# treangenlab/Seqwin

Measured on AMD Instinct MI355X. Metric: Gbp/s minimizer-indexed, higher is better.
Workload: dtype u64

## Files before the change

seqwin_amd/csrc/index.hip:

```cpp
#include <cstdlib>
#include <cstring>
#include <map>
#include <memory>

#include <rocprim/rocprim.hpp>

#include "device.hpp"

namespace sw {

namespace {

constexpr int TPB = 256;
inline unsigned blocks_for(uint64_t n, int per = TPB) { return (unsigned)((n + per - 1) / per); }
inline bool ranks_by_table()
{
    const char *e = SW_TEST_GETENV("SEQWIN_AMD_RANKS");
    return e && !strcmp(e, "table");
}

template <class K, class V>
void sort_pairs(K *&keys, K *&keys_alt, V *&vals, V *&vals_alt, size_t n, unsigned begin_bit, unsigned end_bit,
                hipStream_t stream)
{
    rocprim::double_buffer<K> dk(keys, keys_alt);
    rocprim::double_buffer<V> dv(vals, vals_alt);
    size_t tmp_bytes = 0;
    SW_HIP(rocprim::radix_sort_pairs(nullptr, tmp_bytes, dk, dv, n, begin_bit, end_bit, stream));
    DevArray<unsigned char> tmp(tmp_bytes);
    SW_HIP(rocprim::radix_sort_pairs(tmp.p, tmp_bytes, dk, dv, n, begin_bit, end_bit, stream));
    keys = dk.current();
    keys_alt = dk.alternate();
    vals = dv.current();
    vals_alt = dv.alternate();
}

}

bool sort_keys64_is_own(size_t n)
{
    const char *e = SW_TEST_GETENV("SEQWIN_AMD_SORT");
    const bool own = e ? !strcmp(e, "own") : n >= (1ull << 23);
    return own && !(e && !strcmp(e, "rocprim"));
}

void sort_keys64(uint64_t *&keys, uint64_t *&keys_alt, size_t n, unsigned begin_bit, unsigned end_bit, hipStream_t stream,
                 uint32_t *d_fail, bool perm_hi32, unsigned long long *d_hist_given, unsigned layout_bits)
{
    if (sort_keys64_is_own(n)) {
        radix_sort_keys64(keys, keys_alt, n, begin_bit, end_bit, stream, d_fail, perm_hi32, d_hist_given, layout_bits);
        return;
    }
    rocprim::double_buffer<uint64_t> dk(keys, keys_alt);
    size_t tmp_bytes = 0;
    SW_HIP(rocprim::radix_sort_keys(nullptr, tmp_bytes, dk, n, begin_bit, end_bit, stream));
    DevArray<unsigned char> tmp(tmp_bytes);
    SW_HIP(rocprim::radix_sort_keys(tmp.p, tmp_bytes, dk, n, begin_bit, end_bit, stream));
    keys = dk.current();
    keys_alt = dk.alternate();
}

bool sort_pairs_is_own(size_t n, unsigned bits)
{
    const char *e = SW_TEST_GETENV("SEQWIN_AMD_PAIR_SORT"), *all = SW_TEST_GETENV("SEQWIN_AMD_SORT");
    if (e && !strcmp(e, "rocprim")) return false;
    if (bits % 8 != 0 || bits > 32 || n >= 0xFFFFFFFFull) return false;
    bool own = n >= (1ull << 20);
    if (all) own = !strcmp(all, "own");
    if (e && !strcmp(e, "own")) own = true;
    return own && radix_pairs_available();
}

bool sort_pairs32(uint32_t *&keys, uint32_t *&keys_alt, OccPay *&vals, OccPay *&vals_alt, uint64_t n, unsigned end_bit,
                  hipStream_t stream, uint32_t *d_fail, uint32_t *low_out)
{
    if (sort_pairs_is_own(n, end_bit)) {
        radix_sort_pairs32(keys, keys_alt, vals, vals_alt, n, end_bit, stream, d_fail, nullptr, std::function<void()>(), low_out);
        return low_out != nullptr && n != 0 && end_bit != 0;
    }
    sort_pairs(keys, keys_alt, vals, vals_alt, n, 0, end_bit, stream);
    return false;
}

void check_sort_failed(uint32_t fail_word)
{
    if (fail_word)
        raise(SW_ERR_RUNTIME, "internal error: a radix pass gave up waiting for a lower-numbered workgroup (set SEQWIN_AMD_SORT=rocprim)");
}

namespace {

template <class InIt, class OutIt, class T>
void inclusive_sum(InIt in, OutIt out, size_t n, T, hipStream_t stream)
{
    size_t tmp_bytes = 0;
    SW_HIP(rocprim::inclusive_scan(nullptr, tmp_bytes, in, out, n, rocprim::plus<T>(), stream));
    DevArray<unsigned char> tmp(tmp_bytes);
    SW_HIP(rocprim::inclusive_scan(tmp.p, tmp_bytes, in, out, n, rocprim::plus<T>(), stream));
}

template <class InIt, class OutIt, class T>
void inclusive_sum_keep(InIt in, OutIt out, size_t n, T, hipStream_t stream, DevArray<unsigned char> &tmp)
{
    size_t tmp_bytes = 0;
    SW_HIP(rocprim::inclusive_scan(nullptr, tmp_bytes, in, out, n, rocprim::plus<T>(), stream));
    tmp.alloc(tmp_bytes);
    SW_HIP(rocprim::inclusive_scan(tmp.p, tmp_bytes, in, out, n, rocprim::plus<T>(), stream));
}

template <class InIt, class OutIt, class T>
void exclusive_sum(InIt in, OutIt out, size_t n, T init, hipStream_t stream)
{
    size_t tmp_bytes = 0;
    SW_HIP(rocprim::exclusive_scan(nullptr, tmp_bytes, in, out, init, n, rocprim::plus<T>(), stream));
    DevArray<unsigned char> tmp(tmp_bytes);
    SW_HIP(rocprim::exclusive_scan(tmp.p, tmp_bytes, in, out, init, n, rocprim::plus<T>(), stream));
}

struct U32ToU64 {
    __host__ __device__ uint64_t operator()(uint32_t v) const { return v; }
};

struct HeadFlag {
    const uint64_t *keys;
    uint64_t sentinel;
    __host__ __device__ uint32_t operator()(uint64_t s) const
    {
        const uint64_t k = keys[s];
        return (k != sentinel && (s == 0 || k != keys[s - 1])) ? 1u : 0u;
    }
};

template <bool INDEX, bool RAW = false>
__global__ void k_order(const uint64_t *__restrict__ stage_hash, const uint64_t *__restrict__ stage_kmer,
                        const uint32_t *__restrict__ tile_count, const uint64_t *__restrict__ tile_offset,
                        const uint64_t *__restrict__ dst_off, uint32_t n_tiles, uint64_t mult, uint64_t *__restrict__ hash,
                        uint64_t *__restrict__ kmer, uint32_t *__restrict__ key32, OccPay *__restrict__ pay,
                        uint32_t *__restrict__ rec)
{
    const uint32_t wave = (blockIdx.x * blockDim.x + threadIdx.x) >> 6;
    const uint32_t lane = threadIdx.x & 63u;
    if (wave >= n_tiles) return;
    const uint32_t c = tile_count[wave];
    const uint64_t src = tile_offset[wave], dst = dst_off[wave];
    for (uint32_t i = lane; i < c; i += 64) {
        uint64_t h = stage_hash[src + i];
        if (!RAW) {
            h *= mult;
            h ^= h >> 27;
        }
        const uint64_t km = stage_kmer[src + i];
        if (INDEX) {
            key32[dst + i] = (uint32_t)(h >> 32);
            OccPay p;
            p.low = (uint32_t)h;
            p.pos = (uint32_t)km;
            p.rec = (uint32_t)(km >> 32);
            p.idx = (uint32_t)(dst + i);
            pay[dst + i] = p;
            rec[dst + i] = p.rec;
            if (hash) hash[dst + i] = h;
        } else {
            hash[dst + i] = h;
            kmer[dst + i] = km;
        }
    }
}

__global__ void k_rows_to_pay(const uint64_t *__restrict__ rows, uint64_t n, uint32_t *__restrict__ key32, OccPay *__restrict__ pay)
{
    const uint64_t i = (uint64_t)blockIdx.x * blockDim.x + threadIdx.x;
    if (i >= n) return;
    const uint64_t h = rows[2 * i], km = rows[2 * i + 1];
    key32[i] = (uint32_t)(h >> 32);
    OccPay p;
    p.low = (uint32_t)h;
    p.pos = (uint32_t)km;
    p.rec = (uint32_t)(km >> 32);
    p.idx = (uint32_t)i;
    pay[i] = p;
}

__global__ void k_iota(uint32_t *v, uint64_t n)
{
    const uint64_t i = (uint64_t)blockIdx.x * blockDim.x + threadIdx.x;
    if (i < n) v[i] = (uint32_t)i;
}

#ifndef SW_NODES_ROWS
#define SW_NODES_ROWS 4
#endif
constexpr int NODES_ROWS = SW_NODES_ROWS;
constexpr int NODES_THREADS = 1024;
constexpr int NODES_WAVES = NODES_THREADS / 64;
constexpr uint32_t NODES_ROW = NODES_THREADS * 2;
constexpr uint32_t NODES_TILE = NODES_ROW * NODES_ROWS;
constexpr uint32_t UNSORT_BITS = 14;
constexpr uint32_t UNSORT_RANGE = 1u << UNSORT_BITS;
constexpr bool UNSORT_FUSED_DEFAULT = true;
constexpr uint64_t UNSORT_DIRECT_MAX = 1ull << 25;

constexpr unsigned long long TS_AGG = 1ull << 62, TS_INC = 2ull << 62;

__device__ __forceinline__ unsigned long long interleave32(uint32_t a, uint32_t b)
{
    unsigned long long x = a, y = b;
    x = (x | (x << 16)) & 0x0000FFFF0000FFFFull; y = (y | (y << 16)) & 0x0000FFFF0000FFFFull;
    x = (x | (x << 8)) & 0x00FF00FF00FF00FFull;  y = (y | (y << 8)) & 0x00FF00FF00FF00FFull;
    x = (x | (x << 4)) & 0x0F0F0F0F0F0F0F0Full;  y = (y | (y << 4)) & 0x0F0F0F0F0F0F0F0Full;
    x = (x | (x << 2)) & 0x3333333333333333ull;  y = (y | (y << 2)) & 0x3333333333333333ull;
    x = (x | (x << 1)) & 0x5555555555555555ull;  y = (y | (y << 1)) & 0x5555555555555555ull;
    return x | (y << 1);
}

constexpr uint32_t RANK_REP = 0x80000000u;
constexpr uint8_t OWNER_DROP = 0xFF;
constexpr uint32_t NODES_DIGITS = 256;
struct NodesScat {
    uint64_t stage[NODES_TILE];
    unsigned long long goff[NODES_DIGITS];
    uint32_t cnt[NODES_DIGITS];
    uint32_t lstart[NODES_DIGITS];
};
template <bool BITS, bool REP, bool SCAT = false>
__global__ __launch_bounds__(NODES_THREADS) void k_nodes(const uint32_t *__restrict__ key32, const OccPay *__restrict__ pay, uint64_t n,
                                               uint64_t base, const uint32_t *__restrict__ rec_flag, sw_kmer *__restrict__ kmers,
                                               uint64_t *__restrict__ node_hash, uint32_t *__restrict__ node_start,
                                               uint32_t *__restrict__ rank_direct,
                                               uint64_t *__restrict__ uval,
                                               unsigned long long *__restrict__ tbits, unsigned long long *__restrict__ nbits,
                                               unsigned long long *__restrict__ tile_state, uint32_t *__restrict__ ticket,
                                               uint32_t *__restrict__ n_nodes_out, uint32_t *__restrict__ order_bad,
                                               unsigned long long *__restrict__ cursor, uint32_t dig_shift, uint32_t dig_mask)
{
    __shared__ uint32_t s_tile, s_excl;
    __shared__ uint32_t s_row[NODES_ROWS * NODES_WAVES];
    static_assert(NODES_ROWS * NODES_WAVES <= 128, "the (row, wave) group counts are scanned by one wave, two per lane");
    const uint32_t lane = threadIdx.x & 63u, wave = threadIdx.x >> 6;
    NodesScat *sc = nullptr;
    if constexpr (SCAT) {
        __shared__ NodesScat s_scat;
        sc = &s_scat;
        if (threadIdx.x < NODES_DIGITS) sc->cnt[threadIdx.x] = 0;
    }
    if (threadIdx.x == 0) s_tile = atomicAdd(ticket, 1u);
    __syncthreads();
    const uint32_t tile = s_tile;
    const uint64_t s0 = (uint64_t)tile * NODES_TILE;
    uint32_t k[NODES_ROWS][2], within[NODES_ROWS], headm = 0, prec[NODES_ROWS];
    OccPay p[NODES_ROWS][2];
    unsigned long long misorder = 0;
#pragma unroll
    for (int r = 0; r < NODES_ROWS; ++r) {
        const uint64_t s = s0 + (uint64_t)r * NODES_ROW + 2 * threadIdx.x;
        k[r][0] = k[r][1] = 0;
        p[r][0] = p[r][1] = OccPay{0, 0, 0, 0};
        if (s + 1 < n) {
            const uint2 kk = *reinterpret_cast<const uint2 *>(key32 + s);
            k[r][0] = kk.x;
            k[r][1] = kk.y;
            p[r][0] = pay[s];
            p[r][1] = pay[s + 1];
        } else if (s < n) {
            k[r][0] = key32[s];
            p[r][0] = pay[s];
        }
        uint32_t pk = __shfl_up(k[r][1], 1, 64), plow = __shfl_up(p[r][1].low, 1, 64), pidx = __shfl_up(p[r][1].idx, 1, 64);
        prec[r] = __shfl_up(p[r][1].rec, 1, 64);
        if (lane == 0 && s < n && s) {
            pk = key32[s - 1];
            const OccPay q = pay[s - 1];
            plow = q.low;
            prec[r] = q.rec;
            pidx = q.idx;
        }
        const bool h0 = s < n && (s == 0 || k[r][0] != pk || p[r][0].low != plow);
        const bool h1 = s + 1 < n && (k[r][1] != k[r][0] || p[r][1].low != p[r][0].low);
#ifndef SW_NO_ORDER_GUARD
        {
            const unsigned long long hp = ((unsigned long long)pk << 32) | plow, h0v = ((unsigned long long)k[r][0] << 32) | p[r][0].low,
                                     h1v = ((unsigned long long)k[r][1] << 32) | p[r][1].low;
            const bool bad0 = s < n && s && (h0v < hp || (!h0 && p[r][0].idx <= pidx));
            const bool bad1 = s + 1 < n && (h1v < h0v || (!h1 && p[r][1].idx <= p[r][0].idx));
            misorder |= __ballot(bad0 || bad1);
        }
#else
        (void)pidx;
#endif
        const unsigned long long b0 = __ballot(h0), b1 = __ballot(h1), lt = (1ull << lane) - 1ull;
        within[r] = (uint32_t)__popcll(b0 & lt) + (uint32_t)__popcll(b1 & lt);
        if (h0) headm |= 1u << (2 * r);
        if (h1) headm |= 2u << (2 * r);
        if (lane == 0) s_row[r * NODES_WAVES + wave] = (uint32_t)__popcll(b0) + (uint32_t)__popcll(b1);
    }
    if (misorder && lane == 0) atomicAdd(order_bad, (uint32_t)__popcll(misorder));
    uint32_t drank[NODES_ROWS][2];
    if constexpr (SCAT) {
#pragma unroll
        for (int r = 0; r < NODES_ROWS; ++r)
#pragma unroll
            for (int e = 0; e < 2; ++e) {
                drank[r][e] = 0;
                if (s0 + (uint64_t)r * NODES_ROW + 2 * threadIdx.x + e < n)
                    drank[r][e] = atomicAdd(&sc->cnt[(p[r][e].idx >> dig_shift) & dig_mask], 1u);
            }
    }
    __syncthreads();
    if (SCAT && wave == 1) {
        const uint4 c4 = reinterpret_cast<const uint4 *>(sc->cnt)[lane];
        const uint32_t c[4] = {c4.x, c4.y, c4.z, c4.w};
        unsigned long long g[4];
#pragma unroll
        for (int j = 0; j < 4; ++j)
            g[j] = c[j] ? atomicAdd(&cursor[(size_t)(4 * lane + j) * UNSORT_CURSOR_STRIDE], (unsigned long long)c[j]) : 0ull;
        uint32_t incl = c[0] + c[1] + c[2] + c[3];
        for (uint32_t d = 1; d < 64; d <<= 1) {
            const uint32_t up = __shfl_up(incl, d, 64);
            if (lane >= d) incl += up;
        }
        uint32_t before = incl - (c[0] + c[1] + c[2] + c[3]);
#pragma unroll
        for (int j = 0; j < 4; ++j) {
            sc->lstart[4 * lane + j] = before;
            sc->goff[4 * lane + j] = g[j] - before;
            before += c[j];
        }
    }
    if (wave == 0) {
        constexpr uint32_t GROUPS = NODES_ROWS * NODES_WAVES;
        const uint32_t c0 = (2 * lane < GROUPS) ? s_row[2 * lane] : 0u, c1 = (2 * lane + 1 < GROUPS) ? s_row[2 * lane + 1] : 0u;
        uint32_t incl = c0 + c1;
        for (uint32_t d = 1; d < 64; d <<= 1) {
            const uint32_t up = __shfl_up(incl, d, 64);
            if (lane >= d) incl += up;
        }
        const uint32_t total = __shfl(incl, 63, 64);
        if (2 * lane < GROUPS) s_row[2 * lane] = incl - c0 - c1;
        if (2 * lane + 1 < GROUPS) s_row[2 * lane + 1] = incl - c1;
        if (lane == 0)
            __hip_atomic_store(&tile_state[tile], (tile == 0 ? TS_INC : TS_AGG) | total, __ATOMIC_RELAXED, __HIP_MEMORY_SCOPE_AGENT);
        uint32_t excl = 0;
        if (tile) {
            int64_t look = (int64_t)tile - 1;
            for (;;) {
                const int64_t idx = look - lane;
                const unsigned long long st = idx >= 0 ? __hip_atomic_load(&tile_state[idx], __ATOMIC_RELAXED, __HIP_MEMORY_SCOPE_AGENT)
                                                       : TS_INC;
                const unsigned long long inc = __ballot((st >> 62) == 2), none = __ballot((st >> 62) == 0);
                const uint32_t first_inc = inc ? (uint32_t)__builtin_ctzll(inc) : 64u;
                const unsigned long long needed = first_inc >= 63 ? ~0ull : ((2ull << first_inc) - 1ull);
                if (none & needed) {
                    __builtin_amdgcn_s_sleep(2);
                    continue;
                }
                uint32_t v = (lane <= first_inc) ? (uint32_t)st : 0u;
                for (int d = 32; d; d >>= 1) v += __shfl_xor(v, d, 64);
                excl += v;
                if (first_inc < 64) break;
                look -= 64;
            }
            if (lane == 0)
                __hip_atomic_store(&tile_state[tile], TS_INC | (unsigned long long)(excl + total), __ATOMIC_RELAXED,
                                   __HIP_MEMORY_SCOPE_AGENT);
        }
        if (lane == 0) {
            s_excl = excl;
            if (s0 + NODES_TILE >= n) *n_nodes_out = excl + total;
        }
    }
    __syncthreads();
    const uint32_t excl = s_excl;
    if constexpr (SCAT) {
#pragma unroll
        for (int r = 0; r < NODES_ROWS; ++r)
#pragma unroll
            for (int e = 0; e < 2; ++e) drank[r][e] += sc->lstart[(p[r][e].idx >> dig_shift) & dig_mask];
    }
#pragma unroll
    for (int r = 0; r < NODES_ROWS; ++r) {
        const uint64_t s = s0 + (uint64_t)r * NODES_ROW + 2 * threadIdx.x;
        const bool live0 = s < n, live1 = s + 1 < n;
        const bool h0 = (headm >> (2 * r)) & 1u, h1 = (headm >> (2 * r + 1)) & 1u;
        const uint32_t nid0 = excl + s_row[r * NODES_WAVES + wave] + within[r] + (h0 ? 1u : 0u) - 1u;
        const uint32_t nid1 = nid0 + (h1 ? 1u : 0u);
        uint32_t w0 = nid0, w1 = nid1;
        uint32_t f0 = 0, f1 = 0, pf = 0;
        if (BITS || REP) {
            f0 = live0 ? rec_flag[p[r][0].rec] : 0u;
            f1 = live1 ? rec_flag[p[r][1].rec] : 0u;
            pf = __shfl_up(f1, 1, 64);
            if (lane == 0 && live0 && s) pf = rec_flag[prec[r]];
        }
        if (REP) {
            uint32_t nk = __shfl_down(k[r][0], 1, 64), nlow = __shfl_down(p[r][0].low, 1, 64), nf = __shfl_down(f0, 1, 64);
            bool nlive = __shfl_down((int)live0, 1, 64) != 0;
            if (lane == 63) {
                nlive = s + 2 < n;
                if (nlive) {
                    nk = key32[s + 2];
                    const OccPay q = pay[s + 2];
                    nlow = q.low;
                    nf = rec_flag[q.rec];
                }
            }
            const bool same01 = live1 && !h1 && (f1 >> 1) == (f0 >> 1);
            const bool same_p0 = live0 && !h0 && (f0 >> 1) == (pf >> 1);
            const bool same_1n = live1 && nlive && nk == k[r][1] && nlow == p[r][1].low && (nf >> 1) == (f1 >> 1);
            if (same_p0 || same01) w0 |= RANK_REP;
            if (same01 || same_1n) w1 |= RANK_REP;
        }
        if (live1) {
            *reinterpret_cast<uint4 *>(kmers + s) = make_uint4(p[r][0].pos, p[r][0].rec, p[r][1].pos, p[r][1].rec);
            if (!SCAT && uval)
                *reinterpret_cast<ulonglong2 *>(uval + s) = make_ulonglong2(((uint64_t)p[r][0].idx << 32) | w0,
                                                                          ((uint64_t)p[r][1].idx << 32) | w1);
        } else if (live0) {
            sw_kmer km;
            km.pos = p[r][0].pos;
            km.record_idx = p[r][0].rec;
            kmers[s] = km;
            if (!SCAT && uval) uval[s] = ((uint64_t)p[r][0].idx << 32) | w0;
        }
        if constexpr (SCAT) {
            if (live0) sc->stage[drank[r][0]] = ((uint64_t)p[r][0].idx << 32) | w0;
            if (live1) sc->stage[drank[r][1]] = ((uint64_t)p[r][1].idx << 32) | w1;
        }
        if (rank_direct) {
            if (live0) rank_direct[p[r][0].idx] = w0;
            if (live1) rank_direct[p[r][1].idx] = w1;
        }
#pragma unroll
        for (int e = 0; e < 2; ++e) {
            const bool head = e ? h1 : h0;
            if (head) {
                const uint32_t nid = e ? nid1 : nid0;
                node_hash[nid] = ((uint64_t)k[r][e] << 32) | p[r][e].low;
                node_start[nid] = (uint32_t)(s + e);
            }
        }
        if (BITS) {
            const bool first0 = live0 && (h0 || (f0 >> 1) != (pf >> 1)), first1 = live1 && (h1 || (f1 >> 1) != (f0 >> 1));
            const unsigned long long t0 = __ballot(first0 && (f0 & 1u)), t1 = __ballot(first1 && (f1 & 1u));
            const unsigned long long g0 = __ballot(first0 && !(f0 & 1u)), g1 = __ballot(first1 && !(f1 & 1u));
            if (lane == 0 && live0) {
                const uint64_t wd = s >> 6;
                tbits[wd] = interleave32((uint32_t)t0, (uint32_t)t1);
                nbits[wd] = interleave32((uint32_t)g0, (uint32_t)g1);
                if (s + 64 < n) {
                    tbits[wd + 1] = interleave32((uint32_t)(t0 >> 32), (uint32_t)(t1 >> 32));
                    nbits[wd + 1] = interleave32((uint32_t)(g0 >> 32), (uint32_t)(g1 >> 32));
                }
            }
        }
    }
    if constexpr (SCAT) {
        asm volatile("s_waitcnt lgkmcnt(0)" ::: "memory");
        __builtin_amdgcn_s_barrier();
        asm volatile("" ::: "memory");
        const uint32_t cnt_tile = (uint32_t)min((uint64_t)NODES_TILE, n - s0);
        constexpr int OUT = NODES_TILE / NODES_THREADS;
        uint64_t word[OUT], at[OUT];
#pragma unroll
        for (int j = 0; j < OUT; ++j) word[j] = sc->stage[j * NODES_THREADS + threadIdx.x];
#pragma unroll
        for (int j = 0; j < OUT; ++j) at[j] = sc->goff[(uint32_t)(word[j] >> (32 + dig_shift)) & dig_mask] + (j * NODES_THREADS + threadIdx.x);
#pragma unroll
        for (int j = 0; j < OUT; ++j)
            if (j * NODES_THREADS + threadIdx.x < cnt_tile && at[j] < n) uval[at[j]] = word[j];
    }
}

__device__ __forceinline__ uint32_t popc_range(const unsigned long long *__restrict__ w, uint64_t a, uint64_t b)
{
    if (a >= b) return 0;
    const uint64_t wa = a >> 6, wb = (b - 1) >> 6;
    const unsigned long long ma = ~0ull << (a & 63u), mb = ~0ull >> (63u - ((b - 1) & 63u));
    if (wa == wb) return (uint32_t)__popcll(w[wa] & ma & mb);
    uint32_t c = (uint32_t)__popcll(w[wa] & ma) + (uint32_t)__popcll(w[wb] & mb);
    for (uint64_t i = wa + 1; i < wb; ++i) c += (uint32_t)__popcll(w[i]);
    return c;
}

constexpr int FIN_THREADS = 256;
template <bool BITS>
__global__ __launch_bounds__(FIN_THREADS) void k_finish_nodes(sw_node *__restrict__ nodes, uint64_t n_nodes, const uint64_t *__restrict__ node_hash,
                                                              const uint32_t *__restrict__ node_start, uint64_t base, uint64_t end,
                                                              const unsigned long long *__restrict__ tbits,
                                                              const unsigned long long *__restrict__ nbits, double inv_tar, double inv_neg)
{
    static_assert(sizeof(sw_node) == 40, "five 8-byte words per node");
    __shared__ __align__(16) unsigned long long stage[FIN_THREADS * 5];
    const uint64_t i0 = (uint64_t)blockIdx.x * FIN_THREADS, i = i0 + threadIdx.x;
    if (i < n_nodes) {
        const uint32_t a = node_start[i];
        const uint64_t b = i + 1 < n_nodes ? (uint64_t)node_start[i + 1] : end - base;
        uint32_t n_tar = 0, n_neg = 0;
        double pen = 0.0;
        if (BITS) {
            n_tar = popc_range(tbits, a, b);
            n_neg = popc_range(nbits, a, b);
            {
#pragma clang fp contract(off)
                const double ft = (double)n_tar * inv_tar;
                const double fn = (double)n_neg * inv_neg;
                const double omf = 1.0 - ft;
                const double aa = omf * omf;
                const double bb = fn * fn;
                const double sum = aa + bb;
                pen = __dsqrt_rn(sum);
            }
        }
        unsigned long long *w = stage + threadIdx.x * 5;
        w[0] = node_hash[i];
        w[1] = base + a;
        w[2] = base + b;
        w[3] = ((unsigned long long)n_neg << 32) | n_tar;
        w[4] = (unsigned long long)__double_as_longlong(pen);
    }
    __syncthreads();
    const uint64_t cnt = min((uint64_t)FIN_THREADS, n_nodes - i0);
    const uint32_t n16 = (uint32_t)(cnt * 40 / 16), tail8 = (uint32_t)((cnt * 40) % 16) / 8;
    uint4 *dst = reinterpret_cast<uint4 *>(nodes + i0);
    const uint4 *src = reinterpret_cast<const uint4 *>(stage);
    for (uint32_t t = threadIdx.x; t < n16; t += FIN_THREADS) dst[t] = src[t];
    if (tail8 && threadIdx.x == 0) reinterpret_cast<unsigned long long *>(nodes + i0)[n16 * 2] = stage[n16 * 2];
}

__global__ void k_rec_flag(const uint32_t *__restrict__ rec_asm, const uint8_t *__restrict__ is_target, uint64_t n_records,
                           uint32_t *__restrict__ rec_flag)
{
    const uint64_t r = (uint64_t)blockIdx.x * blockDim.x + threadIdx.x;
    if (r < n_records) {
        const uint32_t a = rec_asm[r];
        rec_flag[r] = (a << 1) | ((is_target && is_target[a]) ? 1u : 0u);
    }
}

constexpr unsigned long long TABLE_EMPTY = ~0ull;
__device__ __forceinline__ uint64_t table_mix(uint64_t x)
{
    return x ^ (x >> 29);
}

__global__ void k_table_build(const sw_node *__restrict__ nodes, uint64_t n_nodes, ulonglong2 *__restrict__ slots, uint64_t mask,
                              uint32_t *__restrict__ rank_of_empty_key)
{
    const uint64_t r = (uint64_t)blockIdx.x * blockDim.x + threadIdx.x;
    if (r >= n_nodes) return;
    const unsigned long long h = nodes[r].hash;
    if (h == TABLE_EMPTY) {
        *rank_of_empty_key = (uint32_t)r;
        return;
    }
    uint64_t s = table_mix(h) & mask;
    for (;;) {
        const unsigned long long old = atomicCAS(&slots[s].x, TABLE_EMPTY, h);
        if (old == TABLE_EMPTY) {
            slots[s].y = r;
            return;
        }
        s = (s + 1) & mask;
    }
}

__global__ void k_table_lookup(const uint64_t *__restrict__ hash, uint64_t n, const ulonglong2 *__restrict__ slots, uint64_t mask,
                               const uint32_t *__restrict__ rank_of_empty_key, uint32_t *__restrict__ rank)
{
    const uint64_t i = (uint64_t)blockIdx.x * blockDim.x + threadIdx.x;
    if (i >= n) return;
    const unsigned long long h = hash[i];
    if (h == TABLE_EMPTY) {
        rank[i] = *rank_of_empty_key;
        return;
    }
    uint64_t s = table_mix(h) & mask;
    for (;;) {
        const ulonglong2 e = slots[s];
        if (e.x == h) {
            rank[i] = (uint32_t)e.y;
            return;
        }
        if (e.x == TABLE_EMPTY) {
            rank[i] = 0xFFFFFFFFu;
            return;
        }
        s = (s + 1) & mask;
    }
}

__global__ __launch_bounds__(1024) void k_unsort_bucket(const uint64_t *__restrict__ uval, uint64_t n, uint32_t *__restrict__ rank)
{
    __shared__ uint32_t sr[UNSORT_RANGE];
    const uint64_t b0 = (uint64_t)blockIdx.x * UNSORT_RANGE;
    const uint32_t cnt = (uint32_t)min((uint64_t)UNSORT_RANGE, n - b0);
#pragma unroll
    for (uint32_t h = 0; h < UNSORT_RANGE / 1024u; h += 8) {
        uint64_t v[8];
#pragma unroll
        for (uint32_t j = 0; j < 8; ++j) {
            const uint32_t t = threadIdx.x + (h + j) * 1024u;
            v[j] = t < cnt ? uval[b0 + t] : 0ull;
        }
#pragma unroll
        for (uint32_t j = 0; j < 8; ++j)
            if (threadIdx.x + (h + j) * 1024u < cnt) sr[(uint32_t)(v[j] >> 32) & (UNSORT_RANGE - 1u)] = (uint32_t)v[j];
    }
    __syncthreads();
    for (uint32_t t = threadIdx.x; t < cnt; t += 1024) rank[b0 + t] = sr[t];
}

__global__ void k_node_starts(const sw_node *__restrict__ nodes, uint64_t n_nodes, uint32_t *__restrict__ start)
{
    const uint64_t i = (uint64_t)blockIdx.x * blockDim.x + threadIdx.x;
    if (i < n_nodes) start[i] = (uint32_t)nodes[i].start;
}

__global__ void k_occ_rows(const sw_kmer *__restrict__ kmers, const sw_node *__restrict__ nodes,
                           const uint32_t *__restrict__ start, uint64_t n_nodes, uint64_t n_kmers, uint64_t rec_offset,
                           uint64_t *__restrict__ rows)
{
    const uint64_t s = (uint64_t)blockIdx.x * blockDim.x + threadIdx.x;
    if (s >= n_kmers) return;
    uint64_t lo = 0, hi = n_nodes;
    while (hi - lo > 1) {
        const uint64_t mid = (lo + hi) >> 1;
        if (start[mid] <= s) lo = mid; else hi = mid;
    }
    rows[2 * s] = nodes[lo].hash;
    rows[2 * s + 1] = (uint64_t)kmers[s].pos | (((uint64_t)kmers[s].record_idx + rec_offset) << 32);
}

__global__ void k_strided_copy(const uint64_t *__restrict__ src, uint32_t stride, uint32_t col, uint64_t n,
                               uint64_t *__restrict__ dst)
{
    const uint64_t i = (uint64_t)blockIdx.x * blockDim.x + threadIdx.x;
    if (i < n) dst[i] = src[i * stride + col];
}

__global__ void k_gather_col(const uint64_t *__restrict__ rows, uint32_t stride, uint32_t col,
                             const uint32_t *__restrict__ idx, uint64_t n, uint64_t *__restrict__ dst)
{
    const uint64_t i = (uint64_t)blockIdx.x * blockDim.x + threadIdx.x;
    if (i < n) dst[i] = rows[(uint64_t)idx[i] * stride + col];
}

__global__ void k_rebase_nodes(sw_node *__restrict__ nodes, uint64_t n_nodes, uint64_t base)
{
    const uint64_t i = (uint64_t)blockIdx.x * blockDim.x + threadIdx.x;
    if (i < n_nodes) {
        nodes[i].start += base;
        nodes[i].stop += base;
    }
}

struct PairHeadFlag {
    const uint64_t *a, *b;
    __host__ __device__ uint32_t operator()(uint64_t s) const
    {
        return (s == 0 || a[s] != a[s - 1] || b[s] != b[s - 1]) ? 1u : 0u;
    }
};

__global__ void k_merge_edge_heads(const uint64_t *__restrict__ f, const uint64_t *__restrict__ sd,
                                   const uint32_t *__restrict__ ecum, uint64_t n, uint64_t *__restrict__ edge_start)
{
    const uint64_t s = (uint64_t)blockIdx.x * blockDim.x + threadIdx.x;
    if (s >= n) return;
    if (s == 0 || f[s] != f[s - 1] || sd[s] != sd[s - 1]) edge_start[ecum[s] - 1] = s;
}

__global__ void k_merge_edges(const uint64_t *__restrict__ f, const uint64_t *__restrict__ sd,
                              const uint64_t *__restrict__ wcum, const uint64_t *__restrict__ edge_start,
                              uint64_t n_edges, uint64_t n, sw_edge *__restrict__ edges)
{
    const uint64_t e = (uint64_t)blockIdx.x * blockDim.x + threadIdx.x;
    if (e >= n_edges) return;
    const uint64_t s = edge_start[e];
    const uint64_t s1 = (e + 1 < n_edges) ? edge_start[e + 1] : n;
    edges[e].first = f[s];
    edges[e].second = sd[s];
    edges[e].weight = wcum[s1 - 1] - (s ? wcum[s - 1] : 0ull);
}

__global__ void k_lower_bounds(const sw_node *__restrict__ nodes, uint64_t n_nodes, uint64_t n_kmers,
                               const sw_edge *__restrict__ edges, uint64_t n_edges, const uint64_t *__restrict__ nb,
                               const uint64_t *__restrict__ eb, uint32_t n_bounds, uint64_t *__restrict__ occ_split,
                               uint64_t *__restrict__ edge_split)
{
    const uint32_t j = blockIdx.x * blockDim.x + threadIdx.x;
    if (j >= n_bounds) return;
    {
        uint64_t lo = 0, hi = n_nodes;
        while (lo < hi) {
            const uint64_t mid = (lo + hi) >> 1;
            if (nodes[mid].hash < nb[j]) lo = mid + 1; else hi = mid;
        }
        occ_split[j] = (lo < n_nodes) ? nodes[lo].start : n_kmers;
    }
    {
        uint64_t lo = 0, hi = n_edges;
        while (lo < hi) {
            const uint64_t mid = (lo + hi) >> 1;
            if (edges[mid].first < eb[j]) lo = mid + 1; else hi = mid;
        }
        edge_split[j] = lo;
    }
}

__global__ void k_pen_flags(const sw_kmer *__restrict__ kmers, uint64_t n, const uint32_t *__restrict__ rec_asm,
                            uint64_t n_records, const uint8_t *__restrict__ is_target, uint64_t *__restrict__ X,
                            uint64_t *__restrict__ Y)
{
    const uint64_t s = (uint64_t)blockIdx.x * blockDim.x + threadIdx.x;
    if (s >= n) return;
    const uint32_t r = kmers[s].record_idx;
    const bool oob = r >= n_records;
    uint64_t x = 0, y = oob ? 1ull : 0ull;
    if (s) {
        const uint32_t rp = kmers[s - 1].record_idx;
        if (r < rp) y |= 1ull << 32;
        if (!oob) {
            const uint32_t a = rec_asm[r];
            const uint32_t ap = (rp < n_records) ? rec_asm[rp] : 0xFFFFFFFFu;
            if (a != ap) x = is_target[a] ? (1ull << 32) : 1ull;
        }
    }
    X[s] = x;
    Y[s] = y;
}

__global__ void k_pen_nodes(const sw_kmer *__restrict__ kmers, uint64_t n_kmers, sw_node *__restrict__ nodes,
                            uint64_t n_nodes, const uint32_t *__restrict__ rec_asm, uint64_t n_records,
                            const uint8_t *__restrict__ is_target, const uint64_t *__restrict__ XS,
                            const uint64_t *__restrict__ YS, double inv_tar, double inv_neg,
                            uint32_t *__restrict__ err)
{
    const uint64_t i = (uint64_t)blockIdx.x * blockDim.x + threadIdx.x;
    if (i >= n_nodes) return;
    const uint64_t start = nodes[i].start, stop = nodes[i].stop;
    if (start == stop) {
        nodes[i].n_tar = 0;
        nodes[i].n_neg = 0;
        nodes[i].penalty = 1.0;
        return;
    }
    if (start > stop || stop > n_kmers) {
        atomicOr(err, 1u);
        return;
    }
    {
        const uint64_t y = YS[stop - 1] - (start ? YS[start - 1] : 0ull);
        if ((uint32_t)y) {
            atomicOr(err, 2u);
            return;
        }
        const uint64_t dec = (YS[stop - 1] - YS[start]) >> 32;
        if (dec) {
            atomicOr(err, 4u);
            return;
        }
    }
    const uint32_t a0 = rec_asm[kmers[start].record_idx];
    const uint64_t x = XS[stop - 1] - XS[start];
    const uint32_t t0 = is_target[a0] ? 1u : 0u;
    const uint32_t n_tar = t0 + (uint32_t)(x >> 32);
    const uint32_t n_neg = (1u - t0) + (uint32_t)x;
    nodes[i].n_tar = n_tar;
    nodes[i].n_neg = n_neg;
    {
#pragma clang fp contract(off)
        const double ft = (double)n_tar * inv_tar;
// ... 544 lines not shown
            if (lane == 0)
                __hip_atomic_store(&tile_state[tile], TS_INC | (unsigned long long)(excl + total), __ATOMIC_RELAXED,
                                   __HIP_MEMORY_SCOPE_AGENT);
        }
        if (lane == 0) {
            s_excl = excl;
            if (t0 + RLE_TILE >= m) {
                *n_runs_out = excl + total;
                ustart[excl + total] = (uint32_t)m;
            }
        }
    }
    __syncthreads();
    const uint32_t base = s_excl + s_wave[wave];
#pragma unroll
    for (int j = 0; j < RLE_ITEMS; ++j)
        if ((headm >> j) & 1u) {
            ukeys[base + below[j]] = k[j];
            ustart[base + below[j]] = (uint32_t)(w0 + (uint64_t)j * 64 + lane);
        }
    (void)cnt;
}

template <bool RUNS = false>
__global__ void k_edges_runs(const uint64_t *__restrict__ ukeys, const uint32_t *__restrict__ usum, unsigned pshift, uint64_t pmask,
                             uint64_t n_edges, unsigned nb, const sw_node *__restrict__ nodes,
                             const uint64_t *__restrict__ rank_hash, sw_edge *__restrict__ edges)
{
    const uint64_t e = (uint64_t)blockIdx.x * blockDim.x + threadIdx.x;
    if (e >= n_edges) return;
    const uint64_t pair = (ukeys[e] >> pshift) & pmask;
    const uint32_t u = (uint32_t)(pair >> nb), v = (uint32_t)(pair & ((1ull << nb) - 1ull));
    edges[e].first = rank_hash ? rank_hash[u] : nodes[u].hash;
    edges[e].second = rank_hash ? rank_hash[v] : nodes[v].hash;
    edges[e].weight = RUNS ? usum[e + 1] - usum[e] : usum[e];
}



__global__ void k_unpermute(const uint32_t *__restrict__ perm, const uint32_t *__restrict__ by_row, uint64_t n,
                            uint32_t *__restrict__ orig)
{
    const uint64_t j = (uint64_t)blockIdx.x * blockDim.x + threadIdx.x;
    if (j < n) orig[perm[j]] = by_row[j];
}

__global__ void k_adj_rows(const uint64_t *__restrict__ kmer, const uint32_t *__restrict__ rank,
                           const uint32_t *__restrict__ rec_asm, uint64_t n, unsigned nb, uint64_t sentinel,
                           uint64_t asm_base, uint64_t *__restrict__ rows)
{
    const uint64_t i = (uint64_t)blockIdx.x * blockDim.x + threadIdx.x;
    if (i + 1 >= n) return;
    const uint32_t r0 = (uint32_t)(kmer[i] >> 32), r1 = (uint32_t)(kmer[i + 1] >> 32);
    if (r0 == r1) {
        uint32_t u = rank[i], v = rank[i + 1];
        if (v < u) { const uint32_t t = u; u = v; v = t; }
        rows[2 * i] = ((uint64_t)u << nb) | v;
        rows[2 * i + 1] = asm_base + rec_asm[r0];
    } else {
        rows[2 * i] = sentinel;
        rows[2 * i + 1] = 0;
    }
}


__global__ void k_adj_rows_packed(const uint64_t *__restrict__ kmer, const uint32_t *__restrict__ rank,
                                  const uint32_t *__restrict__ rec_asm, uint64_t n, unsigned nb, unsigned ab, uint64_t sentinel,
                                  uint64_t asm_base, uint64_t *__restrict__ rows)
{
    const uint64_t i = (uint64_t)blockIdx.x * blockDim.x + threadIdx.x;
    if (i + 1 >= n) return;
    const uint32_t r0 = (uint32_t)(kmer[i] >> 32), r1 = (uint32_t)(kmer[i + 1] >> 32);
    if (r0 == r1) {
        uint32_t u = rank[i], v = rank[i + 1];
        if (v < u) { const uint32_t t = u; u = v; v = t; }
        rows[i] = (((((uint64_t)u << nb) | v)) << ab) | (asm_base + rec_asm[r0]);
    } else {
        rows[i] = sentinel;
    }
}

__global__ void k_split_rows2(const uint64_t *__restrict__ rows, uint64_t n, uint64_t *__restrict__ key,
                              uint32_t *__restrict__ val)
{
    const uint64_t i = (uint64_t)blockIdx.x * blockDim.x + threadIdx.x;
    if (i < n) {
        key[i] = rows[2 * i];
        val[i] = (uint32_t)rows[2 * i + 1];
    }
}

__global__ void k_node_hashes(const sw_node *__restrict__ nodes, uint64_t n_nodes, uint64_t *__restrict__ out)
{
    const uint64_t i = (uint64_t)blockIdx.x * blockDim.x + threadIdx.x;
    if (i < n_nodes) out[i] = nodes[i].hash;
}

__global__ void k_threshold_sums(const sw_node *__restrict__ nodes, uint64_t n, unsigned long long *__restrict__ sums)
{
    const uint64_t i = (uint64_t)blockIdx.x * blockDim.x + threadIdx.x;
    uint64_t a = 0, b = 0, c = 0;
    if (i < n) {
        const uint64_t t = nodes[i].n_tar, g = nodes[i].n_neg;
        a = t;
        b = t * t;
        c = t * g;
    }
    for (int d = 32; d; d >>= 1) {
        a += __shfl_down(a, d, 64);
        b += __shfl_down(b, d, 64);
        c += __shfl_down(c, d, 64);
    }
    if ((threadIdx.x & 63u) == 0) {
        if (a) atomicAdd(&sums[0], (unsigned long long)a);
        if (b) atomicAdd(&sums[1], (unsigned long long)b);
        if (c) atomicAdd(&sums[2], (unsigned long long)c);
    }
}

struct EdgeKeepFlag {
    const sw_edge *edges;
    uint64_t th;
    __host__ __device__ uint32_t operator()(uint64_t e) const { return edges[e].weight > th ? 1u : 0u; }
};

__device__ __forceinline__ uint64_t node_index_of(const sw_node *nodes, uint64_t n_nodes, uint64_t h)
{
    uint64_t lo = 0, hi = n_nodes;
    while (lo < hi) {
        const uint64_t mid = (lo + hi) >> 1;
        if (nodes[mid].hash < h) lo = mid + 1; else hi = mid;
    }
    return lo;
}

__global__ void k_filter_edges(const sw_edge *__restrict__ edges, uint64_t n_edges, uint64_t th,
                               const uint32_t *__restrict__ ecum, const sw_node *__restrict__ nodes, uint64_t n_nodes,
                               sw_edge *__restrict__ out, uint32_t *__restrict__ node_keep)
{
    const uint64_t e = (uint64_t)blockIdx.x * blockDim.x + threadIdx.x;
    if (e >= n_edges || !(edges[e].weight > th)) return;
    out[ecum[e] - 1] = edges[e];
    node_keep[node_index_of(nodes, n_nodes, edges[e].first)] = 1u;
    node_keep[node_index_of(nodes, n_nodes, edges[e].second)] = 1u;
}

__global__ void k_compact_nodes(const sw_node *__restrict__ nodes, uint64_t n_nodes, const uint32_t *__restrict__ keep,
                                const uint32_t *__restrict__ kcum, sw_node *__restrict__ out)
{
    const uint64_t i = (uint64_t)blockIdx.x * blockDim.x + threadIdx.x;
    if (i < n_nodes && keep[i]) out[kcum[i] - 1] = nodes[i];
}

__global__ void k_filter_keep(const sw_node *__restrict__ nodes, uint64_t n_nodes, const uint64_t *__restrict__ used,
                              uint64_t n_used, uint32_t *__restrict__ keep, uint64_t *__restrict__ size)
{
    const uint64_t i = (uint64_t)blockIdx.x * blockDim.x + threadIdx.x;
    if (i >= n_nodes) return;
    const uint64_t h = nodes[i].hash;
    uint64_t lo = 0, hi = n_used;
    while (lo < hi) {
        const uint64_t mid = (lo + hi) >> 1;
        if (used[mid] < h) lo = mid + 1; else hi = mid;
    }
    const bool k = lo < n_used && used[lo] == h;
    keep[i] = k ? 1u : 0u;
    size[i] = k ? nodes[i].stop - nodes[i].start : 0ull;
}

__global__ void k_filter_nodes(const sw_node *__restrict__ nodes, uint64_t n_nodes, const uint32_t *__restrict__ keep,
                               const uint32_t *__restrict__ kcum, const uint64_t *__restrict__ scum,
                               sw_node *__restrict__ nodes_out, uint64_t *__restrict__ src_start,
                               uint64_t *__restrict__ dst_start)
{
    const uint64_t i = (uint64_t)blockIdx.x * blockDim.x + threadIdx.x;
    if (i >= n_nodes || !keep[i]) return;
    const uint32_t o = kcum[i] - 1;
    const uint64_t sz = nodes[i].stop - nodes[i].start;
    const uint64_t ns = scum[i] - sz;
    sw_node nd = nodes[i];
    src_start[o] = nd.start;
    dst_start[o] = ns;
    nd.start = ns;
    nd.stop = ns + sz;
    nodes_out[o] = nd;
}

__global__ void k_filter_kmers(const sw_kmer *__restrict__ kmers, const uint64_t *__restrict__ src_start,
                               const uint64_t *__restrict__ dst_start, uint64_t n_kept, uint64_t n_out,
                               sw_kmer *__restrict__ out)
{
    const uint64_t j = (uint64_t)blockIdx.x * blockDim.x + threadIdx.x;
    if (j >= n_out) return;
    uint64_t lo = 0, hi = n_kept;
    while (hi - lo > 1) {
        const uint64_t mid = (lo + hi) >> 1;
        if (dst_start[mid] <= j) lo = mid; else hi = mid;
    }
    out[j] = kmers[src_start[lo] + (j - dst_start[lo])];
}

__global__ void k_checksum(const sw_kmer *kmers, uint64_t nk, const sw_node *nodes, uint64_t nn, const sw_edge *edges,
                           uint64_t ne, uint64_t kbase, uint64_t nbase, uint64_t ebase, unsigned long long *sums)
{
    const uint64_t i = (uint64_t)blockIdx.x * blockDim.x + threadIdx.x;
    uint64_t a = 0, b = 0, c = 0;
    if (i < nk) a = ck_kmer(kbase + i, kmers[i]);
    if (i < nn) b = ck_node(nbase + i, nodes[i]);
    if (i < ne) c = ck_edge(ebase + i, edges[i]);
    for (int d = 32; d; d >>= 1) {
        a += __shfl_down(a, d, 64);
        b += __shfl_down(b, d, 64);
        c += __shfl_down(c, d, 64);
    }
    if ((threadIdx.x & 63u) == 0) {
        if (a) atomicAdd(&sums[0], (unsigned long long)a);
        if (b) atomicAdd(&sums[1], (unsigned long long)b);
        if (c) atomicAdd(&sums[2], (unsigned long long)c);
    }
}

__global__ void k_verify_nodes(const sw_node *__restrict__ nodes, uint64_t n_nodes, uint64_t n_kmers, uint64_t base,
                               uint64_t n_assemblies, int scored, uint32_t *__restrict__ start_bits,
                               unsigned long long *__restrict__ out)
{
    const uint64_t i = (uint64_t)blockIdx.x * blockDim.x + threadIdx.x;
    if (i >= n_nodes) return;
    const sw_node nd = nodes[i];
    if (i && !(nodes[i - 1].hash < nd.hash)) atomicAdd(&out[0], 1ull);
    const uint64_t prev_stop = i ? nodes[i - 1].stop : base;
    bool bad = nd.start != prev_stop || nd.stop <= nd.start || nd.stop - base > n_kmers;
    if (i == n_nodes - 1 && nd.stop - base != n_kmers) bad = true;
    if (bad) atomicAdd(&out[1], 1ull);
    else atomicOr(&start_bits[(nd.start - base) >> 5], 1u << ((nd.start - base) & 31u));
    if (scored) {
        const uint64_t c = (uint64_t)nd.n_tar + nd.n_neg, size = nd.stop - nd.start;
        if (c < 1 || c > size || c > n_assemblies) atomicAdd(&out[7], 1ull);
    }
}

__global__ void k_verify_kmers(const sw_kmer *__restrict__ kmers, uint64_t n, const uint32_t *__restrict__ start_bits,
                               unsigned long long *__restrict__ out)
{
    const uint64_t s = (uint64_t)blockIdx.x * blockDim.x + threadIdx.x;
    unsigned long long bad = 0, first_of_record = 0;
    if (s < n) {
        const uint64_t cur = ((uint64_t)kmers[s].record_idx << 32) | kmers[s].pos;
        const bool head = (start_bits[s >> 5] >> (s & 31u)) & 1u;
        if (s && !head) {
            const uint64_t prev = ((uint64_t)kmers[s - 1].record_idx << 32) | kmers[s - 1].pos;
            if (!(prev < cur)) bad = 1;
        }
    }
    (void)first_of_record;
    for (int d = 32; d; d >>= 1) bad += __shfl_down(bad, d, 64);
    if ((threadIdx.x & 63u) == 0 && bad) atomicAdd(&out[2], bad);
}

__global__ void k_verify_edges(const sw_edge *__restrict__ edges, uint64_t n_edges, const sw_node *__restrict__ nodes,
                               uint64_t n_nodes, const uint64_t *__restrict__ rank_hash, uint64_t n_rank_hash,
                               uint64_t n_assemblies, unsigned long long *__restrict__ out)
{
    const uint64_t e = (uint64_t)blockIdx.x * blockDim.x + threadIdx.x;
    unsigned long long wsum = 0;
    if (e < n_edges) {
        const sw_edge ed = edges[e];
        if (e) {
            const sw_edge pe = edges[e - 1];
            if (!(pe.first < ed.first || (pe.first == ed.first && pe.second < ed.second))) atomicAdd(&out[3], 1ull);
        }
        if (ed.first > ed.second) atomicAdd(&out[4], 1ull);
        if (ed.weight < 1 || ed.weight > n_assemblies) atomicAdd(&out[5], 1ull);
        wsum = ed.weight;
        for (int side = 0; side < 2; ++side) {
            const uint64_t h = side ? ed.second : ed.first;
            bool found;
            if (rank_hash) {
                uint64_t lo = 0, hi = n_rank_hash;
                while (lo < hi) {
                    const uint64_t mid = (lo + hi) >> 1;
                    if (rank_hash[mid] < h) lo = mid + 1; else hi = mid;
                }
                found = lo < n_rank_hash && rank_hash[lo] == h;
            } else {
                const uint64_t lo = node_index_of(nodes, n_nodes, h);
                found = lo < n_nodes && nodes[lo].hash == h;
            }
            if (!found) atomicAdd(&out[6], 1ull);
        }
    }
    for (int d = 32; d; d >>= 1) wsum += __shfl_down(wsum, d, 64);
    if ((threadIdx.x & 63u) == 0 && wsum) atomicAdd(&out[8], wsum);
}

__global__ void k_rot_keys(uint32_t *__restrict__ key32, uint64_t n, unsigned left)
{
    const uint64_t i = (uint64_t)blockIdx.x * blockDim.x + threadIdx.x;
    if (i < n) {
        const uint32_t k = key32[i];
        key32[i] = (k << left) | (k >> (32u - left));
    }
}

constexpr uint32_t DESC_BLOCK = 1024;

struct PayView {
    using Key = uint32_t;
    using Elem = OccPay;
    uint32_t *key32;
    OccPay *pay;
    __device__ uint32_t key(uint64_t q) const { return key32[q]; }
    __device__ uint64_t low(uint64_t q) const { return pay[q].low; }
    __device__ static uint64_t low_of(const OccPay &v) { return v.low; }
    __device__ void load(uint64_t q, uint32_t &k, OccPay &v) const { k = key32[q]; v = pay[q]; }
    __device__ void store(uint64_t q, uint32_t k, const OccPay &v) const { key32[q] = k; pay[q] = v; }
};
struct LowView {
    using Key = uint32_t;
    const uint32_t *key32;
    const uint32_t *low32;
    __device__ uint32_t key(uint64_t q) const { return key32[q]; }
    __device__ uint64_t low(uint64_t q) const { return low32[q]; }
};
struct EdgeKeyView {
    using Key = uint64_t;
    using Elem = uint64_t;
    uint64_t *keys;
    unsigned low_bits;
    __device__ uint64_t key(uint64_t q) const { return keys[q] >> low_bits; }
    __device__ uint64_t low(uint64_t q) const { return keys[q]; }
    __device__ static uint64_t low_of(const uint64_t &v) { return v; }
    __device__ void load(uint64_t q, uint64_t &k, uint64_t &v) const { v = keys[q]; k = v >> low_bits; }
    __device__ void store(uint64_t q, uint64_t, const uint64_t &v) const { keys[q] = v; }
};

template <class View>
__device__ __forceinline__ uint32_t descents_of_thread(const View &V, typename View::Key kmask, uint64_t n, uint64_t q0, uint32_t *heads = nullptr)
{
    uint32_t m = 0, hm = 0;
    if (heads) *heads = 0;
    if (q0 >= n) return 0;
    typename View::Key kp = q0 ? V.key(q0 - 1) : 0;
    uint64_t lp = q0 ? V.low(q0 - 1) : 0;
#pragma unroll
    for (uint32_t i = 0; i < 4; ++i) {
        const uint64_t q = q0 + i;
        if (q >= n) break;
        const typename View::Key kq = V.key(q);
        const uint64_t lq = V.low(q);
        if (q && (kq & kmask) == (kp & kmask) && (kq < kp || (kq == kp && lq < lp))) m |= 1u << i;
        if (q == 0 || kq != kp || lq != lp) hm |= 1u << i;
        kp = kq;
        lp = lq;
    }
    if (heads) *heads = (uint32_t)__popc(hm);
    return m;
}

__device__ __forceinline__ uint32_t descents_of_thread(const PayView &V, uint32_t kmask, uint64_t n, uint64_t q0, uint32_t *heads = nullptr)
{
    uint32_t m = 0, hm = 0;
    if (heads) *heads = 0;
    if (q0 >= n) return 0;
    uint32_t kq[4];
    uint64_t lq[4];
    if (q0 + 4 <= n) {
        const uint4 kv = *reinterpret_cast<const uint4 *>(V.key32 + q0);
        kq[0] = kv.x; kq[1] = kv.y; kq[2] = kv.z; kq[3] = kv.w;
#pragma unroll
        for (uint32_t i = 0; i < 4; ++i) lq[i] = reinterpret_cast<const uint4 *>(V.pay + q0 + i)->x;
    } else {
#pragma unroll
        for (uint32_t i = 0; i < 4; ++i) {
            kq[i] = (q0 + i < n) ? V.key32[q0 + i] : 0u;
            lq[i] = (q0 + i < n) ? V.pay[q0 + i].low : 0u;
        }
    }
    uint32_t kp = q0 ? V.key32[q0 - 1] : 0;
    uint64_t lp = q0 ? V.pay[q0 - 1].low : 0;
#pragma unroll
    for (uint32_t i = 0; i < 4; ++i) {
        const uint64_t q = q0 + i;
        if (q >= n) break;
        if (q && (kq[i] & kmask) == (kp & kmask) && (kq[i] < kp || (kq[i] == kp && lq[i] < lp))) m |= 1u << i;
        if (q == 0 || kq[i] != kp || lq[i] != lp) hm |= 1u << i;
        kp = kq[i];
        lp = lq[i];
    }
    if (heads) *heads = (uint32_t)__popc(hm);
    return m;
}

__device__ __forceinline__ uint32_t descents_of_thread(const LowView &V, uint32_t kmask, uint64_t n, uint64_t q0, uint32_t *heads = nullptr)
{
    uint32_t m = 0, hm = 0;
    if (heads) *heads = 0;
    if (q0 >= n) return 0;
    uint32_t kq[4], lq[4];
    if (q0 + 4 <= n) {
        const uint4 kv = *reinterpret_cast<const uint4 *>(V.key32 + q0), lv = *reinterpret_cast<const uint4 *>(V.low32 + q0);
        kq[0] = kv.x; kq[1] = kv.y; kq[2] = kv.z; kq[3] = kv.w;
        lq[0] = lv.x; lq[1] = lv.y; lq[2] = lv.z; lq[3] = lv.w;
    } else {
#pragma unroll
        for (uint32_t i = 0; i < 4; ++i) {
            kq[i] = (q0 + i < n) ? V.key32[q0 + i] : 0u;
            lq[i] = (q0 + i < n) ? V.low32[q0 + i] : 0u;
        }
    }
    uint32_t kp = q0 ? V.key32[q0 - 1] : 0, lp = q0 ? V.low32[q0 - 1] : 0;
#pragma unroll
    for (uint32_t i = 0; i < 4; ++i) {
        const uint64_t q = q0 + i;
        if (q >= n) break;
        if (q && (kq[i] & kmask) == (kp & kmask) && (kq[i] < kp || (kq[i] == kp && lq[i] < lp))) m |= 1u << i;
        if (q == 0 || kq[i] != kp || lq[i] != lp) hm |= 1u << i;
        kp = kq[i];
        lp = lq[i];
    }
    if (heads) *heads = (uint32_t)__popc(hm);
    return m;
}

constexpr uint32_t DESC_SLOT = 4;
template <class View>
__global__ __launch_bounds__(256) void k_count_descents(const View V, typename View::Key kmask, uint64_t n, unsigned long long *__restrict__ cnt,
                                                        uint32_t *__restrict__ slot_q, uint32_t *__restrict__ slot_k)
{
    const uint64_t q0 = (uint64_t)blockIdx.x * DESC_BLOCK + threadIdx.x * 4u;
    uint32_t heads = 0;
    const uint32_t m = descents_of_thread(V, kmask, n, q0, &heads);
    const uint32_t c = (uint32_t)__popc(m);
    __shared__ unsigned long long s;
    __shared__ uint32_t s_n, s_q[DESC_SLOT], s_kk[DESC_SLOT];
    if (threadIdx.x == 0) {
        s = 0;
        s_n = 0;
    }
    __syncthreads();
    unsigned long long w = ((unsigned long long)heads << 32) | c;
    for (int d = 32; d; d >>= 1) w += __shfl_down(w, d, 64);
    if ((threadIdx.x & 63u) == 0 && w) atomicAdd(&s, w);
    __syncthreads();
    const uint32_t dc = (uint32_t)s;
    if (threadIdx.x == 0) cnt[blockIdx.x] = s;
    if (dc == 0 || dc > DESC_SLOT) return;
    uint32_t mm = m;
    while (mm) {
        const uint32_t i = (uint32_t)__builtin_ctz(mm);
        mm &= mm - 1;
        const uint32_t at = atomicAdd(&s_n, 1u);
        s_q[at] = (uint32_t)(q0 + i);
        s_kk[at] = (uint32_t)(V.key(q0 + i) & kmask);
    }
    __syncthreads();
    if (threadIdx.x == 0) {
        for (uint32_t i = 1; i < dc; ++i)
            for (uint32_t j = i; j > 0 && s_q[j] < s_q[j - 1]; --j) {
                const uint32_t tq = s_q[j], tk = s_kk[j];
                s_q[j] = s_q[j - 1];
                s_kk[j] = s_kk[j - 1];
                s_q[j - 1] = tq;
                s_kk[j - 1] = tk;
            }
        for (uint32_t i = 0; i < dc; ++i) {
            slot_q[(size_t)blockIdx.x * DESC_SLOT + i] = s_q[i];
            slot_k[(size_t)blockIdx.x * DESC_SLOT + i] = s_kk[i];
        }
    }
}

template <class View>
__global__ __launch_bounds__(256) void k_list_descents(const View V, typename View::Key kmask, uint64_t n,
                                                       const unsigned long long *__restrict__ cnt,
                                                       const unsigned long long *__restrict__ off, uint32_t n_blocks,
                                                       uint32_t *__restrict__ bad, uint32_t cap, uint32_t *__restrict__ bad_q,
                                                       uint32_t cap_q, unsigned long long *__restrict__ n_desc,
                                                       const uint32_t *__restrict__ slot_q, const uint32_t *__restrict__ slot_k)
{
    const uint32_t b = blockIdx.x;
    const uint32_t c_blk = (uint32_t)cnt[b];
    if (b == n_blocks - 1 && threadIdx.x == 0) {
        const unsigned long long tot = off[b] + cnt[b];
        n_desc[0] = tot & 0xFFFFFFFFull;
        n_desc[1] = tot >> 32;
    }
    if (c_blk == 0) return;
    if (c_blk <= DESC_SLOT) {
        if (threadIdx.x < c_blk) {
            const uint32_t at = (uint32_t)off[b] + threadIdx.x;
            if (bad && at < cap) bad[at] = slot_k[(size_t)b * DESC_SLOT + threadIdx.x];
            if (at < cap_q) bad_q[at] = slot_q[(size_t)b * DESC_SLOT + threadIdx.x];
        }
        return;
    }
    const uint64_t q0 = (uint64_t)b * DESC_BLOCK + threadIdx.x * 4u;
    const uint32_t m = descents_of_thread(V, kmask, n, q0);
    const uint32_t c = (uint32_t)__popc(m);
    __shared__ uint32_t wsum[4];
    const uint32_t lane = threadIdx.x & 63u, wave = threadIdx.x >> 6;
    uint32_t incl = c;
    for (uint32_t d = 1; d < 64; d <<= 1) {
        const uint32_t up = __shfl_up(incl, d, 64);
        if (lane >= d) incl += up;
    }
    if (lane == 63) wsum[wave] = incl;
    __syncthreads();
    uint32_t base = (uint32_t)off[b] + (incl - c);
    for (uint32_t i = 0; i < wave; ++i) base += wsum[i];
    uint32_t mm = m;
    while (mm) {
        const uint32_t i = (uint32_t)__builtin_ctz(mm);
        mm &= mm - 1;
        if (base < cap) bad[base] = (uint32_t)(V.key(q0 + i) & kmask);
        if (base < cap_q) bad_q[base] = (uint32_t)(q0 + i);
        ++base;
    }
}

constexpr uint32_t REPAIR_MAX_DESC = 1u << 26;
constexpr uint32_t REPAIR_MAX_MID = 1u << 22;
constexpr uint32_t REPAIR_THREAD_RUN = 6;
constexpr uint32_t REPAIR_MAX_RUN = 2048;
constexpr uint32_t REPAIR_GRID = 2048;

__device__ __forceinline__ uint64_t readlane64(uint64_t v, uint32_t lane)
{
    const uint32_t lo = (uint32_t)__builtin_amdgcn_readlane((int)(uint32_t)v, (int)lane);
    const uint32_t hi = (uint32_t)__builtin_amdgcn_readlane((int)(uint32_t)(v >> 32), (int)lane);
    return ((uint64_t)hi << 32) | lo;
}

__device__ __forceinline__ uint32_t readlane_key(uint32_t v, uint32_t lane) { return (uint32_t)__builtin_amdgcn_readlane((int)v, (int)lane); }
__device__ __forceinline__ uint64_t readlane_key(uint64_t v, uint32_t lane) { return readlane64(v, lane); }

template <class View>
__global__ __launch_bounds__(256) void k_repair_thread(const View V, typename View::Key kmask, uint64_t n, const uint32_t *__restrict__ bad_q,
                                                       const unsigned long long *__restrict__ n_desc, uint32_t *__restrict__ mid,
                                                       uint32_t *__restrict__ n_mid, uint32_t *__restrict__ status)
{
    constexpr uint32_t RT = REPAIR_THREAD_RUN;
    const unsigned long long D = *n_desc;
    if (D > REPAIR_MAX_DESC) {
        if (blockIdx.x == 0 && threadIdx.x == 0) *status = 1u;
        return;
    }
    const uint64_t n_threads = (uint64_t)gridDim.x * blockDim.x;
    for (uint64_t b = (uint64_t)blockIdx.x * blockDim.x + threadIdx.x; b < D; b += n_threads) {
        const uint32_t q = bad_q[b];
        const typename View::Key k = V.key(q) & kmask;
        if (b && (V.key(bad_q[b - 1]) & kmask) == k) continue;
        uint64_t a = q, e = (uint64_t)q + 1;
        while (a > 0 && e - a <= RT && (V.key(a - 1) & kmask) == k) --a;
        while (e < n && e - a <= RT && (V.key(e) & kmask) == k) ++e;
        const uint32_t len = (uint32_t)(e - a);
        if (len > RT) {
            const uint32_t s = atomicAdd(n_mid, 1u);
            if (s < REPAIR_MAX_MID) mid[s] = (uint32_t)b;
            else *status = 1u;
            continue;
        }
        typename View::Key ki[RT];
        typename View::Elem vi[RT];
#pragma unroll
        for (uint32_t i = 0; i < RT; ++i)
            if (i < len) V.load(a + i, ki[i], vi[i]);
        uint32_t rank[RT];
#pragma unroll
        for (uint32_t i = 0; i < RT; ++i) {
            rank[i] = 0;
#pragma unroll
            for (uint32_t j = 0; j < RT; ++j)
                if (i < len && j < len && j != i) {
                    const uint64_t li = View::low_of(vi[i]), lj = View::low_of(vi[j]);
                    rank[i] += (ki[j] < ki[i] || (ki[j] == ki[i] && (lj < li || (lj == li && j < i)))) ? 1u : 0u;
                }
        }
#pragma unroll
        for (uint32_t i = 0; i < RT; ++i)
            if (i < len && rank[i] != i) V.store(a + rank[i], ki[i], vi[i]);
    }
}

template <class View>
__global__ __launch_bounds__(256) void k_repair_wave(const View V, typename View::Key kmask, uint64_t n, const uint32_t *__restrict__ bad_q,
                                                     const unsigned long long *__restrict__ n_desc, const uint32_t *__restrict__ mid,
                                                     const uint32_t *__restrict__ n_mid, uint32_t *__restrict__ big,
                                                     uint32_t *__restrict__ n_big, uint32_t *__restrict__ status)
{
    if (*n_desc > REPAIR_MAX_DESC) return;
    const uint32_t M = min(*n_mid, REPAIR_MAX_MID);
    const uint32_t lane = threadIdx.x & 63u;
    const uint32_t n_waves = gridDim.x * (blockDim.x >> 6);
    for (uint32_t bi = blockIdx.x * (blockDim.x >> 6) + (threadIdx.x >> 6); bi < M; bi += n_waves) {
        const uint32_t q = bad_q[mid[bi]];
        const typename View::Key k = V.key(q) & kmask;
        uint64_t a = q, e = (uint64_t)q + 1;
        bool too_long = false;
        for (;;) {
            const bool match = a >= 1 + (uint64_t)lane && (V.key(a - 1 - lane) & kmask) == k;
            const unsigned long long miss = ~__ballot(match);
            if (miss) {
                a -= (uint64_t)__builtin_ctzll(miss);
                break;
            }
            a -= 64;
            if (e - a > REPAIR_MAX_RUN) { too_long = true; break; }
        }
        while (!too_long) {
            const bool match = e + lane < n && (V.key(e + lane) & kmask) == k;
            const unsigned long long miss = ~__ballot(match);
            if (miss) {
                e += (uint64_t)__builtin_ctzll(miss);
                break;
            }
            e += 64;
            if (e - a > REPAIR_MAX_RUN) too_long = true;
        }
        const uint32_t len = (uint32_t)(e - a);
        if (too_long || len > REPAIR_MAX_RUN) {
            if (lane == 0) *status = 1u;
            continue;
        }
        if (len > 64) {
            if (lane == 0) {
                const uint32_t s = atomicAdd(n_big, 1u);
                big[2 * s] = (uint32_t)a;
                big[2 * s + 1] = len;
            }
            continue;
        }
        typename View::Key ki = 0;
        typename View::Elem vi;
        uint64_t li = 0;
        const bool have = lane < len;
        if (have) {
            V.load(a + lane, ki, vi);
            li = View::low_of(vi);
        }
        uint32_t rank = 0;
        for (uint32_t j = 0; j < len; ++j) {
            const typename View::Key kj = readlane_key(ki, j);
            const uint64_t lj = readlane64(li, j);
            rank += (kj < ki || (kj == ki && (lj < li || (lj == li && j < lane)))) ? 1u : 0u;
        }
        if (have) V.store(a + rank, ki, vi);
    }
}

constexpr uint32_t REPAIR_MAX_VALUES = 12;
template <class View>
__global__ __launch_bounds__(256) void k_repair_sort(const View V, const uint32_t *__restrict__ n_big, const uint32_t *__restrict__ big)
{
    __shared__ typename View::Elem sv[REPAIR_MAX_RUN];
    __shared__ typename View::Key sk[REPAIR_MAX_RUN];
    __shared__ uint16_t srank[REPAIR_MAX_RUN];
    __shared__ typename View::Key w_k[4];
    __shared__ uint32_t w_cnt[4];
    __shared__ uint64_t w_l[4];
    const uint32_t B = *n_big;
    const uint32_t tid = threadIdx.x, lane = tid & 63u, wave = tid >> 6;
    for (uint32_t b = blockIdx.x; b < B; b += gridDim.x) {
        const uint32_t a = big[2 * b], len = big[2 * b + 1];
        __syncthreads();
        for (uint32_t i = tid; i < len; i += blockDim.x) V.load(a + i, sk[i], sv[i]);
        __syncthreads();
        const uint32_t per = (len + 255u) / 256u, i0 = min(len, tid * per), i1 = min(len, i0 + per);
        uint32_t placed = 0;
        typename View::Key last_k = 0;
        uint64_t last_l = 0;
        bool have_last = false;
        for (uint32_t it = 0; it < REPAIR_MAX_VALUES && placed < len; ++it) {
            typename View::Key mk = ~(typename View::Key)0;
            uint64_t ml = ~0ull;
            bool any = false;
            for (uint32_t i = i0; i < i1; ++i) {
                const typename View::Key k = sk[i];
                const uint64_t l = View::low_of(sv[i]);
                if (have_last && !(k > last_k || (k == last_k && l > last_l))) continue;
                if (!any || k < mk || (k == mk && l < ml)) {
                    mk = k;
                    ml = l;
                    any = true;
                }
            }
            for (int d = 32; d; d >>= 1) {
                const typename View::Key ok = __shfl_xor(mk, d, 64);
                const uint64_t ol = __shfl_xor(ml, d, 64);
                const bool oany = __shfl_xor((int)any, d, 64) != 0;
                if (oany && (!any || ok < mk || (ok == mk && ol < ml))) {
                    mk = ok;
                    ml = ol;
                    any = true;
                }
            }
            __syncthreads();
            if (lane == 0) {
                w_k[wave] = mk;
                w_l[wave] = ml;
                w_cnt[wave] = any ? 1u : 0u;
            }
            __syncthreads();
            any = false;
            for (uint32_t w = 0; w < 4; ++w)
                if (w_cnt[w] && (!any || w_k[w] < mk || (w_k[w] == mk && w_l[w] < ml))) {
                    mk = w_k[w];
                    ml = w_l[w];
                    any = true;
                }
            uint32_t c = 0;
            for (uint32_t i = i0; i < i1; ++i) c += (sk[i] == mk && View::low_of(sv[i]) == ml) ? 1u : 0u;
            uint32_t incl = c;
            for (uint32_t d = 1; d < 64; d <<= 1) {
                const uint32_t up = __shfl_up(incl, d, 64);
                if (lane >= d) incl += up;
            }
            __syncthreads();
            if (lane == 63) w_cnt[wave] = incl;
            __syncthreads();
            uint32_t before = placed + incl - c, total = 0;
            for (uint32_t w = 0; w < 4; ++w) {
                if (w < wave) before += w_cnt[w];
                total += w_cnt[w];
            }
            for (uint32_t i = i0; i < i1; ++i)
                if (sk[i] == mk && View::low_of(sv[i]) == ml) srank[i] = (uint16_t)before++;
            placed += total;
            last_k = mk;
            last_l = ml;
            have_last = true;
        }
        __syncthreads();
        if (placed == len) {
            for (uint32_t i = tid; i < len; i += blockDim.x) V.store(a + srank[i], sk[i], sv[i]);
        } else {
            for (uint32_t i = tid; i < len; i += blockDim.x) {
                const typename View::Key ki = sk[i];
                const typename View::Elem vi = sv[i];
                const uint64_t li = View::low_of(vi);
                uint32_t rank = 0;
                for (uint32_t j = 0; j < len; ++j) {
                    const typename View::Key kj = sk[j];
                    const uint64_t lj = View::low_of(sv[j]);
                    rank += (kj < ki || (kj == ki && (lj < li || (lj == li && j < i)))) ? 1u : 0u;
                }
                V.store(a + rank, ki, vi);
            }
        }
    }
}

struct RepairState {
    DevArray<unsigned long long> n_desc;
    DevArray<unsigned long long> blk_cnt, blk_off;
    DevArray<uint32_t> slot_q, slot_k;
    DevArray<uint32_t> bad_q, mid, big, status;
};

template <class View, class Sweep>
void enqueue_repair(const View &V, const Sweep &W, typename View::Key kmask, uint64_t n, uint32_t *bad, uint32_t cap, RepairState &r,
                    hipStream_t stream)
{
    const uint32_t n_blocks = (uint32_t)((n + DESC_BLOCK - 1) / DESC_BLOCK);
    const uint32_t max_desc = (uint32_t)std::min<uint64_t>(REPAIR_MAX_DESC, std::max<uint64_t>(n, 1));
    const uint32_t max_mid = std::min(max_desc, REPAIR_MAX_MID);
    r.bad_q.alloc(max_desc);
    r.mid.alloc(max_mid);
    r.big.alloc(2 * (size_t)max_mid);
    r.n_desc.alloc(2);
    r.status.alloc(3);
    r.blk_cnt.alloc(n_blocks);
    r.blk_off.alloc(n_blocks);
    r.slot_q.alloc((size_t)n_blocks * DESC_SLOT);
    r.slot_k.alloc((size_t)n_blocks * DESC_SLOT);
    SW_HIP(hipMemsetAsync(r.status.p, 0, 12, stream));
    hipLaunchKernelGGL(k_count_descents<Sweep>, dim3(n_blocks), dim3(256), 0, stream, W, kmask, n, r.blk_cnt.p, r.slot_q.p, r.slot_k.p);
    SW_HIP(hipGetLastError());
    exclusive_sum(r.blk_cnt.p, r.blk_off.p, n_blocks, 0ull, stream);
    hipLaunchKernelGGL(k_list_descents<Sweep>, dim3(n_blocks), dim3(256), 0, stream, W, kmask, n, r.blk_cnt.p, r.blk_off.p,
                       n_blocks, bad, cap, r.bad_q.p, max_desc, r.n_desc.p, r.slot_q.p, r.slot_k.p);
    hipLaunchKernelGGL(k_repair_thread<View>, dim3(REPAIR_GRID), dim3(256), 0, stream, V, kmask, n, r.bad_q.p, r.n_desc.p, r.mid.p,
                       r.status.p + 2, r.status.p);
    hipLaunchKernelGGL(k_repair_wave<View>, dim3(REPAIR_GRID), dim3(256), 0, stream, V, kmask, n, r.bad_q.p, r.n_desc.p,
                       (const uint32_t *)r.mid.p, (const uint32_t *)(r.status.p + 2), r.big.p, r.status.p + 1, r.status.p);
    hipLaunchKernelGGL(k_repair_sort<View>, dim3(REPAIR_GRID), dim3(256), 0, stream, V, r.status.p + 1, r.big.p);
    SW_HIP(hipGetLastError());
}

__global__ void k_bad_runs(const uint32_t *__restrict__ bad, uint32_t n_bad, const uint32_t *__restrict__ key32,
                           uint32_t kmask, uint64_t n, uint32_t *__restrict__ run_start, uint32_t *__restrict__ run_len)
{
    const uint32_t i = blockIdx.x * blockDim.x + threadIdx.x;
    if (i >= n_bad) return;
    const uint32_t k = bad[i];
    if (i && bad[i - 1] == k) {
        run_start[i] = 0;
        run_len[i] = 0;
        return;
    }
    uint64_t lo = 0, hi = n;
    while (lo < hi) {
        const uint64_t mid = (lo + hi) >> 1;
        if ((key32[mid] & kmask) < k) lo = mid + 1; else hi = mid;
    }
    const uint64_t a = lo;
    hi = n;
    while (lo < hi) {
        const uint64_t mid = (lo + hi) >> 1;
        if ((key32[mid] & kmask) <= k) lo = mid + 1; else hi = mid;
    }
    run_start[i] = (uint32_t)a;
    run_len[i] = (uint32_t)(lo - a);
}

__global__ void k_gather_sub(const uint32_t *__restrict__ key32, const OccPay *__restrict__ pay,
                             const uint32_t *__restrict__ run_start, const uint64_t *__restrict__ run_off, uint32_t n_bad,
                             uint64_t n_sub, uint64_t *__restrict__ sub_h, OccPay *__restrict__ sub_v,
                             uint32_t *__restrict__ pos)
{
    const uint64_t t = (uint64_t)blockIdx.x * blockDim.x + threadIdx.x;
    if (t >= n_sub) return;
    uint64_t q = t;
    if (run_off) {
        uint32_t lo = 0, hi = n_bad;
        while (hi - lo > 1) {
            const uint32_t mid = (lo + hi) >> 1;
            if (run_off[mid] <= t) lo = mid; else hi = mid;
        }
        q = (uint64_t)run_start[lo] + (t - run_off[lo]);
        pos[t] = (uint32_t)q;
    }
    const OccPay v = pay[q];
    sub_h[t] = ((uint64_t)key32[q] << 32) | v.low;
    sub_v[t] = v;
}

__global__ void k_scatter_sub(const uint64_t *__restrict__ sub_h, const OccPay *__restrict__ sub_v,
                              const uint32_t *__restrict__ pos, uint64_t n_sub, uint32_t *__restrict__ key32,
                              OccPay *__restrict__ pay)
{
    const uint64_t t = (uint64_t)blockIdx.x * blockDim.x + threadIdx.x;
    if (t >= n_sub) return;
    const uint64_t q = pos ? pos[t] : t;
    key32[q] = (uint32_t)(sub_h[t] >> 32);
    pay[q] = sub_v[t];
}

struct PaySort {
    DevArray<uint32_t> key_a, key_b;
    DevArray<OccPay> pay_a, pay_b;
    uint32_t *key32 = nullptr;
    OccPay *pay = nullptr;
    uint64_t n_repaired = 0;
    DevArray<uint32_t> bad;
    RepairState rep;
    uint32_t cap = 0, kmask = ~0u;
    uint64_t n = 0;
    DevArray<uint32_t> fail;
    DevArray<uint32_t> low;
    const uint64_t *rows_src = nullptr;
    OrderedOcc *staged = nullptr;
};

void sort_pay(uint64_t n, hipStream_t stream, PaySort &o)
{
    unsigned bits = 32;
    if (const char *e = SW_TEST_GETENV("SEQWIN_AMD_SORT_KEYBITS")) {
        const int b = atoi(e);
        if (b >= 1 && b <= 32) bits = (unsigned)b;
    }
    o.kmask = ~0u << (32 - bits);
    o.n = n;
    o.key_b.alloc(n);
    o.pay_b.alloc(n);
    uint32_t *keys = o.key_a.p, *keys_alt = o.key_b.p;
    OccPay *vals = o.pay_a.p, *vals_alt = o.pay_b.p;
    bool have_low = false;
    const bool want_low = bits == 32;
    if (o.staged) {
        OrderedOcc &occ = *o.staged;
        StageSource S{};
        S.stage_hash = occ.stage.stage_hash.p;
        S.stage_kmer = occ.stage.stage_kmer.p;
        S.tile_count = occ.stage.tile_count.p;
        S.tile_offset = occ.stage.tile_offset.p;
        S.dst_off = occ.dst_off.p;
        S.n_tiles = occ.stage_tiles;
        S.mult = occ.stage_mult;
        S.rec_out = occ.rec.p;
        o.fail.alloc(1);
        SW_HIP(hipMemsetAsync(o.fail.p, 0, 4, stream));
        if (want_low) o.low.alloc(n);
        have_low = want_low && n != 0;
        radix_sort_pairs32(keys, keys_alt, vals, vals_alt, n, 32, stream, o.fail.p, &S, [&] {
            occ.stage = SketchOut();
            occ.dst_off.release();
            occ.staged = false;
            o.key_a.alloc(n);
            o.pay_a.alloc(n);
            keys = o.key_a.p;
            vals = o.pay_a.p;
        }, o.low.p);
        o.staged = nullptr;
    } else if (o.rows_src) {
        StageSource S{};
        S.rows = o.rows_src;
        o.fail.alloc(1);
        SW_HIP(hipMemsetAsync(o.fail.p, 0, 4, stream));
        if (want_low) o.low.alloc(n);
        have_low = want_low && n != 0;
        radix_sort_pairs32(keys, keys_alt, vals, vals_alt, n, 32, stream, o.fail.p, &S, [&] {
            o.key_a.alloc(n);
            o.pay_a.alloc(n);
            keys = o.key_a.p;
            vals = o.pay_a.p;
        }, o.low.p);
    } else {
        if (bits < 32) {
            hipLaunchKernelGGL(k_rot_keys, dim3(blocks_for(n)), dim3(TPB), 0, stream, keys, n, bits);
            SW_HIP(hipGetLastError());
        }
        o.fail.alloc(1);
        SW_HIP(hipMemsetAsync(o.fail.p, 0, 4, stream));
        if (want_low && sort_pairs_is_own(n, bits)) o.low.alloc(n);
        have_low = sort_pairs32(keys, keys_alt, vals, vals_alt, n, bits, stream, o.fail.p, o.low.p);
        if (bits < 32) {
            hipLaunchKernelGGL(k_rot_keys, dim3(blocks_for(n)), dim3(TPB), 0, stream, keys, n, 32 - bits);
            SW_HIP(hipGetLastError());
        }
    }
    o.key32 = keys;
    o.pay = vals;
    o.cap = (uint32_t)std::min<uint64_t>(n, std::max<uint64_t>(1u << 16, n / 16));
    o.bad.alloc(o.cap);
    if (have_low) enqueue_repair(PayView{keys, vals}, LowView{keys, o.low.p}, o.kmask, n, o.bad.p, o.cap, o.rep, stream);
    else enqueue_repair(PayView{keys, vals}, PayView{keys, vals}, o.kmask, n, o.bad.p, o.cap, o.rep, stream);
}

bool sort_pay_settle(PaySort &o, unsigned long long D, uint32_t status, hipStream_t stream)
{
    if (D == 0 || status == 0) {
        o.n_repaired = D;
        return false;
    }
    const uint64_t n = o.n;
    const uint32_t kmask = o.kmask, cap = o.cap;
    uint32_t *keys = o.key32;
    OccPay *vals = o.pay;
    DevArray<uint32_t> &bad = o.bad;
    uint64_t n_sub = n;
    DevArray<uint32_t> run_start, run_len, pos;
    DevArray<uint64_t> run_off;
    const bool listed = D <= cap;
    if (listed) {
        const uint32_t nb = (uint32_t)D;
        run_start.alloc(nb);
        run_len.alloc(nb);
        run_off.alloc((size_t)nb + 1);
        hipLaunchKernelGGL(k_bad_runs, dim3((unsigned)blocks_for(nb)), dim3(TPB), 0, stream, bad.p, nb, keys, kmask, n,
                           run_start.p, run_len.p);
        SW_HIP(hipGetLastError());
        exclusive_sum(rocprim::make_transform_iterator(run_len.p, U32ToU64()), run_off.p, nb, (uint64_t)0, stream);
        uint64_t last_off = 0;
        uint32_t last_len = 0;
        SW_HIP(hipMemcpyAsync(&last_off, run_off.p + (nb - 1), 8, hipMemcpyDeviceToHost, stream));
        SW_HIP(hipMemcpyAsync(&last_len, run_len.p + (nb - 1), 4, hipMemcpyDeviceToHost, stream));
        SW_HIP(hipStreamSynchronize(stream));
        n_sub = last_off + last_len;
        pos.alloc(n_sub);
    }
    DevArray<uint64_t> sh0(n_sub), sh1(n_sub);
    DevArray<OccPay> sp0(n_sub), sp1(n_sub);
    hipLaunchKernelGGL(k_gather_sub, dim3(blocks_for(n_sub)), dim3(TPB), 0, stream, keys, vals, run_start.p,
                       listed ? run_off.p : (const uint64_t *)nullptr, (uint32_t)(listed ? D : 0), n_sub, sh0.p, sp0.p, pos.p);
    SW_HIP(hipGetLastError());
    uint64_t *sk = sh0.p, *sk_alt = sh1.p;
    OccPay *sv = sp0.p, *sv_alt = sp1.p;
    sort_pairs(sk, sk_alt, sv, sv_alt, n_sub, 0, 64, stream);
    hipLaunchKernelGGL(k_scatter_sub, dim3(blocks_for(n_sub)), dim3(TPB), 0, stream, sk, sv,
                       listed ? pos.p : (const uint32_t *)nullptr, n_sub, keys, vals);
    SW_HIP(hipGetLastError());
    SW_HIP(hipStreamSynchronize(stream));
    o.n_repaired = n_sub;
    return true;
}

uint64_t settle_sort(PaySort &ps, hipStream_t stream)
{
    uint32_t status = 0, failed = 0;
    unsigned long long dh[2] = {0, 0};
    SW_HIP(hipMemcpyAsync(&status, ps.rep.status.p, 4, hipMemcpyDeviceToHost, stream));
    SW_HIP(hipMemcpyAsync(dh, ps.rep.n_desc.p, 16, hipMemcpyDeviceToHost, stream));
    if (ps.fail.p) SW_HIP(hipMemcpyAsync(&failed, ps.fail.p, 4, hipMemcpyDeviceToHost, stream));
    SW_HIP(hipStreamSynchronize(stream));
    check_sort_failed(failed);
    sort_pay_settle(ps, dh[0], status, stream);
    return dh[1];
}

struct UnsortHold {
    DevArray<uint64_t> a, b;
    const uint64_t *sorted = nullptr;
};
struct NodeParts {
    DevArray<uint64_t> hash;
    DevArray<uint32_t> start;
};
void finish_nodes(sw_index &ix, const NodeParts &np, uint64_t base, uint64_t end, const unsigned long long *tbits,
                  const unsigned long long *nbits, double inv_tar, double inv_neg, hipStream_t stream)
{
    if (!ix.n_nodes) return;
    const dim3 grid((unsigned)((ix.n_nodes + FIN_THREADS - 1) / FIN_THREADS));
    if (tbits && nbits)
        hipLaunchKernelGGL(k_finish_nodes<true>, grid, dim3(FIN_THREADS), 0, stream, ix.nodes.p, ix.n_nodes, (const uint64_t *)np.hash.p,
                           (const uint32_t *)np.start.p, base, end, tbits, nbits, inv_tar, inv_neg);
    else
        hipLaunchKernelGGL(k_finish_nodes<false>, grid, dim3(FIN_THREADS), 0, stream, ix.nodes.p, ix.n_nodes, (const uint64_t *)np.hash.p,
                           (const uint32_t *)np.start.p, base, end, (const unsigned long long *)nullptr,
                           (const unsigned long long *)nullptr, 0.0, 0.0);
    SW_HIP(hipGetLastError());
}

__global__ void k_restore_stream(const uint32_t *__restrict__ key32, const OccPay *__restrict__ pay, uint64_t n, uint64_t *__restrict__ key64,
                                 OccPay *__restrict__ out, uint32_t *__restrict__ bad)
{
    const uint64_t i = (uint64_t)blockIdx.x * blockDim.x + threadIdx.x;
    if (i >= n) return;
    const OccPay q = pay[i];
    if (q.idx >= n) {
        atomicAdd(bad, 1u);
        return;
    }
    key64[q.idx] = ((uint64_t)key32[i] << 32) | q.low;
    out[q.idx] = q;
}
__global__ void k_split_restored(const uint64_t *__restrict__ key64, const OccPay *__restrict__ pay, uint64_t n, uint32_t *__restrict__ key32,
                                 uint32_t *__restrict__ bad)
{
    const uint64_t i = (uint64_t)blockIdx.x * blockDim.x + threadIdx.x;
    if (i >= n) return;
    key32[i] = (uint32_t)(key64[i] >> 32);
    if (pay[i].idx == 0xFFFFFFFFu) atomicAdd(bad, 1u);
}
void resort_pay_stable(PaySort &ps, uint64_t n, hipStream_t stream)
{
    OccPay *cur = ps.pay, *other = (ps.pay == ps.pay_a.p) ? ps.pay_b.p : ps.pay_a.p;
    if (!other || !cur) raise(SW_ERR_RUNTIME, "internal error: the node sort's second buffer is gone");
    DevArray<uint64_t> k0(n), k1(n);
    DevArray<uint32_t> bad(1);
    SW_HIP(hipMemsetAsync(bad.p, 0, 4, stream));
    SW_HIP(hipMemsetAsync(other, 0xFF, n * sizeof(OccPay), stream));
    hipLaunchKernelGGL(k_restore_stream, dim3(blocks_for(n)), dim3(TPB), 0, stream, ps.key32, cur, n, k0.p, other, bad.p);
    SW_HIP(hipGetLastError());
    uint64_t *k = k0.p, *k_alt = k1.p;
    OccPay *v = other, *v_alt = cur;
    sort_pairs(k, k_alt, v, v_alt, n, 0, 64, stream);
    hipLaunchKernelGGL(k_split_restored, dim3(blocks_for(n)), dim3(TPB), 0, stream, k, v, n, ps.key32, bad.p);
    SW_HIP(hipGetLastError());
    uint32_t nbad = 0;
    SW_HIP(hipMemcpyAsync(&nbad, bad.p, 4, hipMemcpyDeviceToHost, stream));
    SW_HIP(hipStreamSynchronize(stream));
    if (nbad) raise(SW_ERR_RUNTIME, "internal error: the node sort lost %u occurrences (not a permutation of its input)", nbad);
    ps.pay = v;
}
uint32_t group_occurrences(PaySort &ps, uint64_t n, uint64_t base, const uint32_t *rec_flag, hipStream_t stream, sw_index &ix,
                           uint32_t *rank_out, DevArray<unsigned long long> *tbits, DevArray<unsigned long long> *nbits,
                           bool *rep_marked = nullptr, UnsortHold *hold = nullptr, NodeParts *parts = nullptr)
{
    sort_pay(n, stream, ps);
    const uint64_t node_cap = settle_sort(ps, stream);
    ix.nodes.alloc(node_cap);
    NodeParts own_parts;
    NodeParts &np = parts ? *parts : own_parts;
    np.hash.alloc(node_cap);
    np.start.alloc(node_cap);
    uint64_t direct_max = UNSORT_DIRECT_MAX;
    if (const char *e = SW_TEST_GETENV("SEQWIN_AMD_UNSORT_DIRECT")) direct_max = 1ull << std::min(40, std::max(0, atoi(e)));
    const bool direct = rank_out && n <= direct_max;
    DevArray<uint64_t> uv0, uv1;
    if (rank_out && !direct) uv0.alloc(n);
    const bool bits = rec_flag && tbits && nbits;
    const bool rep = rec_flag && rep_marked && rank_out && node_cap < (1ull << 31);
    if (rep_marked) *rep_marked = rep;
    if (bits) {
        tbits->alloc((n + 63) / 64);
        nbits->alloc((n + 63) / 64);
    }
    const unsigned blocks = (unsigned)((n + NODES_TILE - 1) / NODES_TILE);
    DevArray<unsigned long long> tile_state(blocks);
    DevArray<uint32_t> words(4);
    uint32_t back[3] = {0, 0, 0};
    if (rank_out && !direct) uv1.alloc(n);
    unsigned nbit = 1;
    while (nbit < 32 && (1ull << nbit) < n) ++nbit;
    bool want_fused = UNSORT_FUSED_DEFAULT;
    if (const char *e = SW_TEST_GETENV("SEQWIN_AMD_UNSORT_FUSED")) want_fused = atoi(e) != 0;
    UnsortPerm perm;
    const char *route = !rank_out ? "none" : direct ? "direct" : nbit <= UNSORT_BITS ? "one bucket" : "sort";
    for (int attempt = 0;; ++attempt) {
        SW_HIP(hipMemsetAsync(tile_state.p, 0, (size_t)blocks * 8, stream));
        SW_HIP(hipMemsetAsync(words.p, 0, 16, stream));
        const bool fused = want_fused && rank_out && !direct && nbit > UNSORT_BITS && sort_keys64_is_own(n) &&
                           radix_unsort_perm_begin(perm, n, UNSORT_BITS, nbit, stream);
        {
            auto launch = [&](auto kern) {
                hipLaunchKernelGGL(kern, dim3(blocks), dim3(NODES_THREADS), 0, stream, ps.key32, ps.pay, n, base, rec_flag, ix.kmers.p,
                                   np.hash.p, np.start.p, direct ? rank_out : (uint32_t *)nullptr, fused ? uv1.p : uv0.p,
                                   bits ? tbits->p : (unsigned long long *)nullptr, bits ? nbits->p : (unsigned long long *)nullptr,
                                   tile_state.p, words.p, words.p + 1, words.p + 3, fused ? perm.cur_a.p : (unsigned long long *)nullptr,
                                   fused ? perm.low_bits + 8 : 0u, fused ? (1u << perm.hi_bits) - 1u : 0u);
            };
            if (fused) {
                if (bits && rep) launch(k_nodes<true, true, true>);
                else if (bits) launch(k_nodes<true, false, true>);
                else if (rep) launch(k_nodes<false, true, true>);
                else launch(k_nodes<false, false, true>);
            } else if (bits && rep) launch(k_nodes<true, true>);
            else if (bits) launch(k_nodes<true, false>);
            else if (rep) launch(k_nodes<false, true>);
            else launch(k_nodes<false, false>);
        }
        SW_HIP(hipGetLastError());
        if (rank_out && !direct) {
            uint64_t *v = uv0.p;
            if (fused) {
                radix_unsort_perm_second(perm, uv1.p, uv0.p, n, stream, words.p + 2);
                route = "fused";
            } else if (nbit > UNSORT_BITS) {
                uint64_t *v_alt = uv1.p;
                if (sort_keys64_is_own(n) && radix_unsort_perm(v, v_alt, n, UNSORT_BITS, nbit, stream, words.p + 2)) route = "two passes";
                else sort_keys64(v, v_alt, n, 32 + UNSORT_BITS, 32 + nbit, stream, words.p + 2, true);
            }
            if (hold && rep && nbit > UNSORT_BITS && !SW_TEST_GETENV("SEQWIN_AMD_ADJ_SEPARATE")) {
                hold->sorted = v;
            } else {
                hipLaunchKernelGGL(k_unsort_bucket, dim3((unsigned)((n + UNSORT_RANGE - 1) / UNSORT_RANGE)), dim3(1024), 0, stream, v, n,
                                   rank_out);
                SW_HIP(hipGetLastError());
            }
        }
        SW_HIP(hipMemcpyAsync(back, words.p + 1, 12, hipMemcpyDeviceToHost, stream));
        SW_HIP(hipStreamSynchronize(stream));
        if (getenv("SEQWIN_AMD_DEBUG_NODES"))
            fprintf(stderr, "[nodes] %llu occurrences (indices of %u bits), attempt %d: unsort route %s, %u nodes, order guard %u\n",
                    (unsigned long long)n, nbit, attempt, route, back[0], back[2]);
        if (back[2] == 0) break;
        if (attempt)
            raise(SW_ERR_RUNTIME, "internal error: the node sort is still out of order after the rocPRIM re-sort (%u places)", back[2]);
        order_guard_tripped(0, back[2]);
        radix_demote_rank();
        resort_pay_stable(ps, n, stream);
    }
    const uint32_t n_nodes = back[0];
    check_sort_failed(back[1]);
    if (n_nodes > node_cap) raise(SW_ERR_RUNTIME, "internal error: %u nodes exceed the bound %llu", n_nodes, (unsigned long long)node_cap);
    ix.n_nodes = n_nodes;
    if (!parts) {
        finish_nodes(ix, np, base, base + n, nullptr, nullptr, 0.0, 0.0, stream);
        SW_HIP(hipStreamSynchronize(stream));
    }
    if (hold && hold->sorted) {
        hold->a = std::move(uv0);
        hold->b = std::move(uv1);
    }
    return n_nodes;
}

void ranks_from_table(const sw_index &ix, const uint64_t *hash, uint64_t n, hipStream_t stream, uint32_t *rank)
{
    uint64_t cap = 1024;
    while (cap < 2 * ix.n_nodes) cap <<= 1;
    DevArray<ulonglong2> slots(cap);
    DevArray<uint32_t> special(1);
    SW_HIP(hipMemsetAsync(slots.p, 0xFF, cap * sizeof(ulonglong2), stream));
    SW_HIP(hipMemsetAsync(special.p, 0xFF, 4, stream));
    if (ix.n_nodes)
        hipLaunchKernelGGL(k_table_build, dim3(blocks_for(ix.n_nodes)), dim3(TPB), 0, stream, ix.nodes.p, ix.n_nodes, slots.p, cap - 1,
                           special.p);
    hipLaunchKernelGGL(k_table_lookup, dim3(blocks_for(n)), dim3(TPB), 0, stream, hash, n, slots.p, cap - 1, special.p, rank);
    SW_HIP(hipGetLastError());
    SW_HIP(hipStreamSynchronize(stream));
}

__global__ void k_append_chunk(const uint32_t *__restrict__ key32, const OccPay *__restrict__ pay, const uint32_t *__restrict__ rec,
                               uint64_t n, uint32_t occ_base, uint32_t rec_base, uint32_t *__restrict__ key32_out,
                               OccPay *__restrict__ pay_out, uint32_t *__restrict__ rec_out)
{
    const uint64_t i = (uint64_t)blockIdx.x * blockDim.x + threadIdx.x;
    if (i >= n) return;
    OccPay p = pay[i];
    p.rec += rec_base;
    p.idx += occ_base;
    key32_out[occ_base + i] = key32[i];
    pay_out[occ_base + i] = p;
    rec_out[occ_base + i] = rec[i] + rec_base;
}

}

void concat_occ(std::vector<OrderedOcc> &chunks, const std::vector<uint64_t> &rec_base, hipStream_t stream, OrderedOcc &out)
{
    uint64_t n = 0;
    for (const OrderedOcc &c : chunks) n += c.n;
    if (n > occ_cap()) raise_occ_cap(n, "minimizer occurrences");
    out.n = n;
    out.key32.alloc(n);
    out.pay.alloc(n);
    out.rec.alloc(n);
    uint64_t at = 0;
    for (size_t c = 0; c < chunks.size(); ++c) {
        OrderedOcc &ch = chunks[c];
        if (ch.n) {
            hipLaunchKernelGGL(k_append_chunk, dim3(blocks_for(ch.n)), dim3(TPB), 0, stream, ch.key32.p, ch.pay.p, ch.rec.p, ch.n,
                               (uint32_t)at, (uint32_t)rec_base[c], out.key32.p, out.pay.p, out.rec.p);
            SW_HIP(hipGetLastError());
        }
        at += ch.n;
        ch = OrderedOcc();
    }
    if (chunks.size() > 1) {
        SW_HIP(hipStreamSynchronize(stream));
        dev_pool_trim();
    }
}

namespace {

struct MinTree {
    const uint64_t *lvl[7];
    uint64_t size[7];
    int levels;
};
constexpr uint64_t LW_NONE = ~0ull;

__global__ void k_lw_level(const uint64_t *__restrict__ in, uint64_t n_in, uint64_t *__restrict__ out, uint64_t n_out)
{
    const uint64_t node = ((uint64_t)blockIdx.x * blockDim.x + threadIdx.x) >> 6;
    const uint32_t lane = threadIdx.x & 63u;
    if (node >= n_out) return;
    const uint64_t i = node * 64 + lane;
    uint64_t v = i < n_in ? in[i] : ~0ull;
    for (int d = 32; d; d >>= 1) {
        const uint64_t o = __shfl_xor(v, d, 64);
        v = o < v ? o : v;
    }
    if (lane == 0) out[node] = v;
}

__device__ uint64_t lw_nearest_left(const MinTree &T, uint64_t i, uint64_t lo, uint64_t h)
{
    uint64_t pos = i, q = 0;
    int t = 0;
    for (;;) {
        const uint64_t gstart = pos & ~63ull, lo_t = lo >> (6 * t), stop = gstart > lo_t ? gstart : lo_t;
        bool found = false;
        for (q = pos; q > stop;) {
            --q;
            if (T.lvl[t][q] < h) {
                found = true;
                break;
            }
        }
        if (found) break;
        if (gstart <= lo_t || t + 1 >= T.levels) return LW_NONE;
        pos >>= 6;
        ++t;
    }
    while (t > 0) {
        const uint64_t cfirst = q << 6, clo = lo >> (6 * (t - 1));
        uint64_t c = cfirst + 64 < T.size[t - 1] ? cfirst + 64 : T.size[t - 1];
        const uint64_t stop = cfirst > clo ? cfirst : clo;
        bool found = false;
        while (c > stop) {
            --c;
            if (T.lvl[t - 1][c] < h) {
                found = true;
                break;
            }
        }
        if (!found) return LW_NONE;
        q = c;
        --t;
    }
    return q;
}

__device__ uint64_t lw_nearest_right(const MinTree &T, uint64_t i, uint64_t hi, uint64_t h)
{
    uint64_t pos = i, q = 0;
    int t = 0;
    for (;;) {
        const uint64_t gend = (pos | 63ull) + 1, hi_t = (hi + ((1ull << (6 * t)) - 1)) >> (6 * t);
        uint64_t stop = gend < hi_t ? gend : hi_t;
        if (T.size[t] < stop) stop = T.size[t];
        bool found = false;
        for (q = pos + 1; q < stop; ++q)
            if (T.lvl[t][q] <= h) {
                found = true;
                break;
            }
        if (found) break;
        if (gend >= hi_t || gend >= T.size[t] || t + 1 >= T.levels) return LW_NONE;
        pos >>= 6;
        ++t;
    }
    while (t > 0) {
        const uint64_t cfirst = q << 6, chi = (hi + ((1ull << (6 * (t - 1))) - 1)) >> (6 * (t - 1));
        uint64_t stop = cfirst + 64 < T.size[t - 1] ? cfirst + 64 : T.size[t - 1];
        if (chi < stop) stop = chi;
        uint64_t c = cfirst;
        bool found = false;
        for (; c < stop; ++c)
            if (T.lvl[t - 1][c] <= h) {
                found = true;
                break;
            }
        if (!found) return LW_NONE;
        q = c;
        --t;
    }
    return q;
}

__global__ void k_lw_index(const uint64_t *__restrict__ kmer, uint64_t c, const uint32_t *__restrict__ rec_seg_off,
                           const uint32_t *__restrict__ seg_pos, const uint32_t *__restrict__ seg_idx, uint32_t *__restrict__ g)
{
    const uint64_t i = (uint64_t)blockIdx.x * blockDim.x + threadIdx.x;
    if (i >= c) return;
    const uint32_t pos = (uint32_t)kmer[i], rec = (uint32_t)(kmer[i] >> 32);
    uint32_t a = rec_seg_off[rec], b = rec_seg_off[rec + 1];
    while (b - a > 1) {
        const uint32_t mid = (a + b) >> 1;
        if (seg_pos[mid] <= pos) a = mid; else b = mid;
    }
    g[i] = seg_idx[a] + (pos - seg_pos[a]);
}

__global__ void k_lw_select(const MinTree T, const uint64_t *__restrict__ kmer, const uint32_t *__restrict__ g, uint64_t c,
                            const uint32_t *__restrict__ rec_nvalid, uint32_t w, uint32_t *__restrict__ keep)
{
    const uint64_t i = (uint64_t)blockIdx.x * blockDim.x + threadIdx.x;
    if (i >= c) return;
    const uint64_t h = T.lvl[0][i];
    const uint32_t rec = (uint32_t)(kmer[i] >> 32);
    const int64_t n = rec_nvalid[rec], gi = g[i];
    uint32_t k = 0;
    if (n >= (int64_t)w && h != ~0ull) {
        uint64_t lo = 0, hi = i;
        while (lo < hi) {
            const uint64_t mid = (lo + hi) >> 1;
            if ((uint32_t)(kmer[mid] >> 32) < rec) lo = mid + 1; else hi = mid;
        }
        uint64_t a = i + 1;
        hi = c;
        while (a < hi) {
            const uint64_t mid = (a + hi) >> 1;
            if ((uint32_t)(kmer[mid] >> 32) <= rec) a = mid + 1; else hi = mid;
        }
        const uint64_t jl = lw_nearest_left(T, i, lo, h), jr = lw_nearest_right(T, i, hi, h);
        const int64_t Lg = jl == LW_NONE ? -1 : (int64_t)g[jl], Rg = jr == LW_NONE ? n : (int64_t)g[jr];
        int64_t x_lo = Lg + 1, x_hi = Rg - (int64_t)w;
        if (gi - (int64_t)w + 1 > x_lo) x_lo = gi - (int64_t)w + 1;
        if (x_lo < 0) x_lo = 0;
        if (gi < x_hi) x_hi = gi;
        if (n - (int64_t)w < x_hi) x_hi = n - (int64_t)w;
        k = x_lo <= x_hi ? 1u : 0u;
    }
    keep[i] = k;
}

template <bool INDEX>
__global__ void k_lw_emit(const uint64_t *__restrict__ canon, const uint64_t *__restrict__ kmer, const uint32_t *__restrict__ keep,
                          const uint64_t *__restrict__ dst, uint64_t c, uint64_t mult, uint64_t *__restrict__ hash,
                          uint64_t *__restrict__ kmer_out, uint32_t *__restrict__ key32, OccPay *__restrict__ pay,
                          uint32_t *__restrict__ rec, unsigned long long *__restrict__ total)
{
    const uint64_t i = (uint64_t)blockIdx.x * blockDim.x + threadIdx.x;
    if (i >= c) return;
    if (i == c - 1) *total = dst[i] + keep[i];
    if (!keep[i]) return;
    const uint64_t d = dst[i], km = kmer[i];
    uint64_t h = canon[i] * mult;
    h ^= h >> 27;
    if (INDEX) {
        key32[d] = (uint32_t)(h >> 32);
        OccPay p;
        p.low = (uint32_t)h;
        p.pos = (uint32_t)km;
        p.rec = (uint32_t)(km >> 32);
        p.idx = (uint32_t)d;
        pay[d] = p;
        rec[d] = p.rec;
        if (hash) hash[d] = h;
    } else {
        hash[d] = h;
        kmer_out[d] = km;
    }
}

}

static bool stage_fits_sort(uint64_t n, uint32_t n_tiles)
{
    if (const char *e = SW_TEST_GETENV("SEQWIN_AMD_ORDER")) {
        if (!strcmp(e, "copy")) return false;
        if (!strcmp(e, "stage")) return n > 0 && radix_pairs_available() && !SW_TEST_GETENV("SEQWIN_AMD_SORT_KEYBITS");
    }
    return n > 0 && sort_pairs_is_own(n, 32) && !SW_TEST_GETENV("SEQWIN_AMD_SORT_KEYBITS") && n / 16 >= n_tiles;
}

__global__ void k_fill_u64(uint64_t *p, uint32_t n, uint64_t v)
{
    if (threadIdx.x < n) p[threadIdx.x] = v;
}

void order_tuples(SketchOut &sk, const Plan &plan, hipStream_t stream, OrderedOcc &out, bool index_form, bool take_stage)
{
    const bool large = plan.w_full > plan.w;
    out.n = sk.n_occ;
    out.staged = false;
    if (!large && out.n > occ_cap()) raise_occ_cap(out.n, "minimizer occurrences");
    const bool table_ranks = index_form && ranks_by_table();
    if (take_stage && index_form && !large && !table_ranks && plan.n_tiles && stage_fits_sort(sk.n_occ, plan.n_tiles)) {
        out.rec.alloc(out.n);
        out.dst_off.alloc((size_t)plan.n_tiles + STAGE_PAD);
        exclusive_sum(rocprim::make_transform_iterator(sk.tile_count.p, U32ToU64()), out.dst_off.p, plan.n_tiles, (uint64_t)0, stream);
        hipLaunchKernelGGL(k_fill_u64, dim3(1), dim3(64), 0, stream, out.dst_off.p + plan.n_tiles, STAGE_PAD, out.n);
        SW_HIP(hipGetLastError());
        out.stage = std::move(sk);
        out.stage_tiles = plan.n_tiles;
        out.stage_mult = plan.mult;
        out.staged = true;
        return;
    }
    auto alloc_out = [&](uint64_t n) {
        if (index_form) {
            out.key32.alloc(n);
            out.pay.alloc(n);
            out.rec.alloc(n);
            if (table_ranks) out.hash.alloc(n);
        } else {
            out.hash.alloc(n);
            out.kmer.alloc(n);
        }
    };
    if (!large) alloc_out(out.n);
    if (plan.n_tiles == 0 || sk.n_occ == 0) {
        out.n = 0;
// ... 172 lines not shown
        const PackedPairEq eq{pshift, pmask};
        size_t tmp_bytes = 0;
        SW_HIP(rocprim::reduce_by_key(nullptr, tmp_bytes, keys, flags, m, ukeys.p, usum.p, ucount.p, rocprim::plus<uint32_t>(), eq,
                                      stream));
        DevArray<unsigned char> tmp(tmp_bytes);
        SW_HIP(rocprim::reduce_by_key(tmp.p, tmp_bytes, keys, flags, m, ukeys.p, usum.p, ucount.p, rocprim::plus<uint32_t>(), eq,
                                      stream));
        hipLaunchKernelGGL(k_drop_sentinel_run, dim3(1), dim3(1), 0, stream, ukeys.p, sentinel, ucount.p);
        SW_HIP(hipGetLastError());
        uint32_t n_edges = 0, failed = 0;
        SW_HIP(hipMemcpyAsync(&n_edges, ucount.p, 4, hipMemcpyDeviceToHost, stream));
        SW_HIP(hipMemcpyAsync(&failed, sort_fail.p, 4, hipMemcpyDeviceToHost, stream));
        SW_HIP(hipStreamSynchronize(stream));
        check_sort_failed(failed);
        ix.n_edges = n_edges;
    }
    if (ix.n_edges == 0) return;
    ix.edges.alloc(ix.n_edges);
    hipLaunchKernelGGL(k_edges_runs<false>, dim3(blocks_for(ix.n_edges)), dim3(TPB), 0, stream, ukeys.p, usum.p, pshift, pmask,
                       (uint64_t)ix.n_edges, nb, ix.nodes.p, rank_hash, ix.edges.p);
    SW_HIP(hipGetLastError());
    SW_HIP(hipStreamSynchronize(stream));
}
}

namespace {
constexpr uint64_t EDGE_BUCKET_MIN_KEYS = 1ull << 26;
constexpr uint32_t EDGE_BUCKET_CAP = 1u << 20, EDGE_BUCKET_SLOTS = 4096;
struct WideKeys {
    unsigned lo_bits, hi_bits;
    uint64_t lo_base;
    RankHash hash;
};
void edges_from_pairs(uint64_t *keys, uint64_t *keys_alt, uint64_t m, uint64_t sentinel, unsigned nb, unsigned ab,
                      uint64_t *ck, uint32_t *ca, const unsigned long long *d_n_cand, uint64_t host_n_cand,
                      const uint64_t *rank_hash, hipStream_t stream, sw_index &ix, hipEvent_t rank_hash_ready = nullptr,
                      unsigned long long *d_hist = nullptr, const WideKeys *wide = nullptr)
{
    ix.n_edges = 0;
    if (m == 0) return;
    const unsigned key_bits = wide ? wide->lo_bits + wide->hi_bits : 2 * nb;
    DevArray<uint32_t> sort_fail(1);
    SW_HIP(hipMemsetAsync(sort_fail.p, 0, 4, stream));
    unsigned low_bits = 0, skip = 0, digit_bits = 0, n_passes = 0;
    if (sort_keys64_is_own(m)) {
        radix_layout(key_bits, &digit_bits, &n_passes);
        const unsigned hb = wide ? wide->hi_bits : nb;
        skip = hb >= digit_bits + 8 ? 1 : 0;
        if (skip && hb >= 2 * digit_bits + 8 && ix.n_nodes && m <= 4 * ix.n_nodes) skip = 2;
        if (const char *e = SW_TEST_GETENV("SEQWIN_AMD_EDGE_SKIP_PASSES")) skip = (unsigned)atoi(e);
        skip = std::min(skip, n_passes - 1);
        low_bits = skip * digit_bits;
    }
    DevArray<uint64_t> ukeys(m);
    DevArray<uint32_t> ucnt(m + 1), ucount(2);
    unsigned long long n_cand = host_n_cand;
    bool by_buckets = !wide && nb < 32 && sort_keys64_is_own(m) && m >= EDGE_BUCKET_MIN_KEYS && ix.n_nodes && m > 4 * ix.n_nodes;
    uint32_t bucket_cap = EDGE_BUCKET_CAP, bucket_slots = EDGE_BUCKET_SLOTS;
    if (const char *e = SW_TEST_GETENV("SEQWIN_AMD_EDGE_SORT")) by_buckets = !wide && nb < 32 && !strcmp(e, "bucket");
    if (const char *e = SW_TEST_GETENV("SEQWIN_AMD_EDGE_BUCKET_CAP")) bucket_cap = (uint32_t)strtoul(e, nullptr, 10);
    if (const char *e = SW_TEST_GETENV("SEQWIN_AMD_EDGE_BUCKET_SLOTS")) bucket_slots = (uint32_t)strtoul(e, nullptr, 10);
    if (by_buckets) {
        unsigned db = 0, np = 0;
        radix_layout(key_bits, &db, &np);
        uint32_t n_runs = 0;
        by_buckets = radix_edge_buckets(keys, keys_alt, m, key_bits, sentinel, d_hist ? d_hist + ((size_t)(np - 1) << db) : nullptr, bucket_cap,
                                        bucket_slots, ukeys.p, ucnt.p, &n_runs, stream, sort_fail.p,
                                        getenv("SEQWIN_AMD_DEBUG_EDGE_REPAIR") != nullptr) == 0;
        if (by_buckets) {
            uint32_t failed = 0;
            SW_HIP(hipMemcpyAsync(&failed, sort_fail.p, 4, hipMemcpyDeviceToHost, stream));
            if (d_n_cand) SW_HIP(hipMemcpyAsync(&n_cand, d_n_cand, 8, hipMemcpyDeviceToHost, stream));
            SW_HIP(hipStreamSynchronize(stream));
            check_sort_failed(failed);
            ix.n_edges = n_runs;
        }
    }
    if (!by_buckets)
        sort_keys64(keys, keys_alt, m, low_bits, key_bits, stream, sort_fail.p, false,
                    d_hist ? d_hist + ((size_t)skip << digit_bits) : nullptr, key_bits);
    RepairState rep;
    if (low_bits && !by_buckets) enqueue_repair(EdgeKeyView{keys, low_bits}, EdgeKeyView{keys, low_bits}, ~0ull, m, nullptr, 0, rep, stream);
    bool demoted = false;
    for (int attempt = 0; !by_buckets; ++attempt) {
        SW_HIP(hipMemsetAsync(ucount.p + 1, 0, 4, stream));
        {
            const unsigned blocks = (unsigned)((m + RLE_TILE - 1) / RLE_TILE);
            DevArray<unsigned long long> tile_state(blocks);
            DevArray<uint32_t> ticket(1);
            SW_HIP(hipMemsetAsync(tile_state.p, 0, (size_t)blocks * 8, stream));
            SW_HIP(hipMemsetAsync(ticket.p, 0, 4, stream));
            hipLaunchKernelGGL(k_rle_keys, dim3(blocks), dim3(RLE_THREADS), 0, stream, (const uint64_t *)keys, m, ukeys.p, ucnt.p, tile_state.p,
                               ticket.p, ucount.p, ucount.p + 1);
            SW_HIP(hipGetLastError());
        }
        hipLaunchKernelGGL(k_drop_sentinel_run, dim3(1), dim3(1), 0, stream, ukeys.p, sentinel, ucount.p);
        SW_HIP(hipGetLastError());
        uint32_t n_edges = 0, failed = 0, left = 0, descents = 0;
        SW_HIP(hipMemcpyAsync(&n_edges, ucount.p, 4, hipMemcpyDeviceToHost, stream));
        SW_HIP(hipMemcpyAsync(&descents, ucount.p + 1, 4, hipMemcpyDeviceToHost, stream));
        SW_HIP(hipMemcpyAsync(&failed, sort_fail.p, 4, hipMemcpyDeviceToHost, stream));
        if (low_bits && attempt == 0) SW_HIP(hipMemcpyAsync(&left, rep.status.p, 4, hipMemcpyDeviceToHost, stream));
        if (d_n_cand) SW_HIP(hipMemcpyAsync(&n_cand, d_n_cand, 8, hipMemcpyDeviceToHost, stream));
        SW_HIP(hipStreamSynchronize(stream));
        check_sort_failed(failed);
        if (low_bits && attempt == 0 && getenv("SEQWIN_AMD_DEBUG_EDGE_REPAIR")) {
            unsigned long long nd[2] = {0, 0};
            uint32_t st[2] = {0, 0};
            SW_HIP(hipMemcpy(nd, rep.n_desc.p, 16, hipMemcpyDeviceToHost));
            SW_HIP(hipMemcpy(st, rep.status.p, 8, hipMemcpyDeviceToHost));
            fprintf(stderr, "[edge repair] %llu keys, %u low bits: %llu descents, %u long runs, leftovers %u\n", (unsigned long long)m, low_bits,
                    nd[0], st[1], st[0]);
        }
        if (left) {
            sort_keys64(keys, keys_alt, m, 0, key_bits, stream, sort_fail.p);
            continue;
        }
        if (descents) {
            if (demoted)
                raise(SW_ERR_RUNTIME, "internal error: the edge keys are still out of order after the ballot-ranked re-sort (%u places)", descents);
            order_guard_tripped(1, descents);
            radix_demote_rank();
            demoted = true;
            sort_keys64(keys, keys_alt, m, 0, key_bits, stream, sort_fail.p);
            continue;
        }
        ix.n_edges = n_edges;
        break;
    }
    if (ix.n_edges == 0) return;
    ix.edges.alloc(ix.n_edges);
    if (rank_hash_ready) SW_HIP(hipStreamWaitEvent(stream, rank_hash_ready, 0));
    if (wide)
        hipLaunchKernelGGL(k_edges_runs_wide<true>, dim3(blocks_for(ix.n_edges)), dim3(TPB), 0, stream, ukeys.p, ucnt.p, (uint64_t)ix.n_edges,
                           wide->hi_bits, wide->lo_base, wide->hash, ix.edges.p);
    else
        hipLaunchKernelGGL(k_edges_runs<true>, dim3(blocks_for(ix.n_edges)), dim3(TPB), 0, stream, ukeys.p, ucnt.p, 0u, ~0ull,
                           (uint64_t)ix.n_edges, nb, ix.nodes.p, rank_hash, ix.edges.p);
    SW_HIP(hipGetLastError());
    if (n_cand) {
        const uint64_t c = n_cand;
        DevArray<uint64_t> ck1(c);
        DevArray<uint32_t> ca1(c);
        uint32_t *a = ca, *a_alt = ca1.p;
        uint64_t *k = ck, *k_alt = ck1.p;
        sort_pairs(a, a_alt, k, k_alt, c, 0, ab, stream);
        sort_pairs(k, k_alt, a, a_alt, c, 0, key_bits, stream);
        DevArray<uint64_t> rkeys(c);
        DevArray<uint32_t> rdups(c), rcount(1);
        auto flags = rocprim::make_transform_iterator(rocprim::make_counting_iterator<uint64_t>(0), RepeatFlag{k, a});
        size_t tmp_bytes = 0;
        SW_HIP(rocprim::reduce_by_key(nullptr, tmp_bytes, k, flags, c, rkeys.p, rdups.p, rcount.p, rocprim::plus<uint32_t>(),
                                      rocprim::equal_to<uint64_t>(), stream));
        DevArray<unsigned char> tmp(tmp_bytes);
        SW_HIP(rocprim::reduce_by_key(tmp.p, tmp_bytes, k, flags, c, rkeys.p, rdups.p, rcount.p, rocprim::plus<uint32_t>(),
                                      rocprim::equal_to<uint64_t>(), stream));
        uint32_t n_runs = 0;
        SW_HIP(hipMemcpyAsync(&n_runs, rcount.p, 4, hipMemcpyDeviceToHost, stream));
        SW_HIP(hipStreamSynchronize(stream));
        if (n_runs) {
            hipLaunchKernelGGL(k_subtract_repeats, dim3(blocks_for(n_runs)), dim3(TPB), 0, stream, rkeys.p, rdups.p, n_runs, ukeys.p,
                               (uint64_t)ix.n_edges, ix.edges.p);
            SW_HIP(hipGetLastError());
        }
    }
    SW_HIP(hipStreamSynchronize(stream));
}

void edges_from_adjacency(uint64_t *keys, uint64_t *keys_alt, uint32_t *vals, uint32_t *vals_alt, uint64_t m,
                          uint64_t sentinel, unsigned nb, const uint64_t *rank_hash, hipStream_t stream, sw_index &ix)
{
    ix.n_edges = 0;
    if (m == 0) return;
    sort_pairs(keys, keys_alt, vals, vals_alt, m, 0, 2 * nb, stream);
    DevArray<uint64_t> ukeys(m);
    DevArray<uint32_t> usum(m);
    DevArray<uint32_t> ucount(1);
    {
        auto flags = rocprim::make_transform_iterator(rocprim::make_counting_iterator<uint64_t>(0), AsmChangeAny{keys, vals});
        size_t tmp_bytes = 0;
        SW_HIP(rocprim::reduce_by_key(nullptr, tmp_bytes, keys, flags, m, ukeys.p, usum.p, ucount.p, rocprim::plus<uint32_t>(),
                                      rocprim::equal_to<uint64_t>(), stream));
        DevArray<unsigned char> tmp(tmp_bytes);
        SW_HIP(rocprim::reduce_by_key(tmp.p, tmp_bytes, keys, flags, m, ukeys.p, usum.p, ucount.p, rocprim::plus<uint32_t>(),
                                      rocprim::equal_to<uint64_t>(), stream));
        hipLaunchKernelGGL(k_drop_sentinel_run, dim3(1), dim3(1), 0, stream, ukeys.p, sentinel, ucount.p);
        SW_HIP(hipGetLastError());
        uint32_t n_edges = 0;
        SW_HIP(hipMemcpyAsync(&n_edges, ucount.p, 4, hipMemcpyDeviceToHost, stream));
        SW_HIP(hipStreamSynchronize(stream));
        ix.n_edges = n_edges;
    }
    if (ix.n_edges == 0) return;
    ix.edges.alloc(ix.n_edges);
    hipLaunchKernelGGL(k_edges_runs<false>, dim3(blocks_for(ix.n_edges)), dim3(TPB), 0, stream, ukeys.p, usum.p, 0u, ~0ull,
                       (uint64_t)ix.n_edges, nb, ix.nodes.p, rank_hash, ix.edges.p);
    SW_HIP(hipGetLastError());
    SW_HIP(hipStreamSynchronize(stream));
}
}

__global__ void k_pack_export_nodes(const sw_node *__restrict__ nodes, uint64_t n, uint64_t n_kmers, uint64_t per, uint32_t *__restrict__ out,
                                    uint64_t *__restrict__ bases, uint32_t *__restrict__ flag)
{
    const uint64_t i = (uint64_t)blockIdx.x * blockDim.x + threadIdx.x;
    if (i >= n) return;
    const sw_node nd = nodes[i];
    const uint64_t cnt = nd.stop - nd.start, next = i + 1 < n ? nodes[i + 1].start : n_kmers;
    uint64_t pen;
    memcpy(&pen, &nd.penalty, 8);
    if (nd.stop < nd.start || cnt > 0xFFFFFFFFull || next != nd.stop || (i == 0 && nd.start != 0) || nd.n_tar || nd.n_neg || pen) atomicOr(flag, 1u);
    out[3 * i] = (uint32_t)nd.hash;
    out[3 * i + 1] = (uint32_t)(nd.hash >> 32);
    out[3 * i + 2] = (uint32_t)cnt;
    if (i % per == 0) bases[i / per] = nd.start;
}
__global__ void k_pack_export_edges(const sw_edge *__restrict__ edges, uint64_t n, uint32_t *__restrict__ out, uint32_t *__restrict__ flag)
{
    const uint64_t i = (uint64_t)blockIdx.x * blockDim.x + threadIdx.x;
    if (i >= n) return;
    const sw_edge e = edges[i];
    if (e.weight > 0xFFFFFFFFull) atomicOr(flag, 1u);
    out[5 * i] = (uint32_t)e.first;
    out[5 * i + 1] = (uint32_t)(e.first >> 32);
    out[5 * i + 2] = (uint32_t)e.second;
    out[5 * i + 3] = (uint32_t)(e.second >> 32);
    out[5 * i + 4] = (uint32_t)e.weight;
}
void pack_export(const sw_node *nodes, uint64_t n_nodes, uint64_t n_kmers, const sw_edge *edges, uint64_t n_edges, uint64_t per, uint32_t *pn,
                 uint64_t *bases, uint32_t *pe, uint32_t *flag, hipStream_t stream)
{
    hipLaunchKernelGGL(k_pack_export_nodes, dim3(blocks_for(n_nodes)), dim3(TPB), 0, stream, nodes, n_nodes, n_kmers, per, pn, bases, flag);
    SW_HIP(hipGetLastError());
    hipLaunchKernelGGL(k_pack_export_edges, dim3(blocks_for(n_edges)), dim3(TPB), 0, stream, edges, n_edges, pe, flag);
    SW_HIP(hipGetLastError());
    SW_HIP(hipStreamSynchronize(stream));
}

void device_get_penalty(const sw_kmer *d_kmers, uint64_t n_kmers, sw_node *d_nodes, uint64_t n_nodes,
                        const uint32_t *d_rec_asm, uint64_t n_records, const uint8_t *d_is_target,
                        uint64_t n_targets, uint64_t n_non_targets, hipStream_t stream, uint64_t *err_flags_host)
{
    PenaltyJob job;
    penalty_launch(d_kmers, n_kmers, d_nodes, n_nodes, d_rec_asm, n_records, d_is_target, n_targets, n_non_targets,
                   stream, job);
    *err_flags_host = penalty_finish(job);
}

void slice_get_penalty(sw_index &ix, uint64_t kmer_base, const uint32_t *d_rec_asm, uint64_t n_records, const uint8_t *d_is_target,
                       uint64_t n_targets, uint64_t n_non_targets, hipStream_t stream, uint64_t *err_flags_host)
{
    *err_flags_host = 0;
    if (!ix.n_nodes) return;
    hipLaunchKernelGGL(k_rebase_nodes, dim3(blocks_for(ix.n_nodes)), dim3(TPB), 0, stream, ix.nodes.p, ix.n_nodes, (uint64_t)0 - kmer_base);
    SW_HIP(hipGetLastError());
    struct Restore {
        sw_index &ix;
        uint64_t base;
        hipStream_t st;
        ~Restore()
        {
            hipLaunchKernelGGL(k_rebase_nodes, dim3(blocks_for(ix.n_nodes)), dim3(TPB), 0, st, ix.nodes.p, ix.n_nodes, base);
            (void)hipGetLastError();
            (void)hipStreamSynchronize(st);
        }
    } restore{ix, kmer_base, stream};
    device_get_penalty(ix.kmers.p, ix.n_kmers, ix.nodes.p, ix.n_nodes, d_rec_asm, n_records, d_is_target, n_targets, n_non_targets,
                       stream, err_flags_host);
}

void build_index(const uint32_t *d_rec_asm, uint64_t n_records, uint64_t n_assemblies, OrderedOcc &occ,
                 const uint8_t *d_is_target, uint64_t n_targets, uint64_t n_non_targets, hipStream_t stream, sw_index &ix)
{
    const uint64_t n = occ.n;
    if (n > occ_cap()) raise_occ_cap(n, "minimizer occurrences");
    Event ev[6];
    SW_HIP(hipEventRecord(ev[0], stream));

    ix.n_kmers = n;
    ix.kmers.alloc(n);
    DevArray<uint32_t> rank(n);
    const bool want_counts = d_is_target != nullptr;
    const bool check_order = want_counts && SW_TEST_GETENV("SEQWIN_AMD_CHECK_ORDER") != nullptr;
    const bool by_table = occ.hash.p != nullptr;
    const bool pair_edges = !SW_TEST_GETENV("SEQWIN_AMD_NO_PACKED_EDGES") && !by_table;
    bool rep_marked = false;
    DevArray<uint32_t> rec_flag;
    DevArray<unsigned long long> tbits, nbits;
    NodeParts parts;
    UnsortHold unsort_hold;
    if (n) {
        const bool bits = want_counts && !check_order;
        if (bits || pair_edges) {
            rec_flag.alloc(n_records);
            hipLaunchKernelGGL(k_rec_flag, dim3(blocks_for(n_records)), dim3(TPB), 0, stream, d_rec_asm, bits ? d_is_target : nullptr,
                               n_records, rec_flag.p);
            SW_HIP(hipGetLastError());
        }
        PaySort ps;
        ps.key_a = std::move(occ.key32);
        ps.pay_a = std::move(occ.pay);
        if (occ.staged) ps.staged = &occ;
        group_occurrences(ps, n, 0, rec_flag.p, stream, ix, by_table ? nullptr : rank.p, bits ? &tbits : nullptr,
                          bits ? &nbits : nullptr, pair_edges ? &rep_marked : nullptr, pair_edges ? &unsort_hold : nullptr, &parts);
        if (!bits || by_table) {
            finish_nodes(ix, parts, 0, n, nullptr, nullptr, 0.0, 0.0, stream);
            if (by_table) ranks_from_table(ix, occ.hash.p, n, stream, rank.p);
        }
    } else {
        ix.n_nodes = 0;
        ix.nodes.alloc(0);
    }
    SW_HIP(hipEventRecord(ev[1], stream));

    PenaltyJob pen;
    hipStream_t side = side_stream();
    bool forked = false;
    if (want_counts && ix.n_nodes) {
        alloc_fork(side);
        forked = true;
        SW_HIP(hipStreamWaitEvent(side, ev[1], 0));
        SW_HIP(hipEventRecord(ev[4], side));
        if (check_order) {
            penalty_launch(ix.kmers.p, n, ix.nodes.p, ix.n_nodes, d_rec_asm, n_records, d_is_target, n_targets, n_non_targets,
                           side, pen);
        } else {
            finish_nodes(ix, parts, 0, n, tbits.p, nbits.p, 1.0 / (double)n_targets, 1.0 / (double)n_non_targets, side);
        }
        SW_HIP(hipEventRecord(ev[5], side));
    }
    SW_HIP(hipEventRecord(ev[2], stream));

    ix.n_edges = 0;
    if (n >= 2) {
        const uint64_t m = n - 1;
        unsigned nb = 1;
        while (((1ull << nb) - 1ull) < ix.n_nodes) ++nb;
        unsigned ab = 1;
        while ((1ull << ab) < n_assemblies) ++ab;
        const unsigned adj_blocks = (unsigned)((n + 1023) / 1024);
        const uint64_t sentinel = (nb == 32) ? ~0ull : ((1ull << (2 * nb)) - 1ull);
        DevArray<uint64_t> k0(m), k1(m);
        if (rep_marked) {
            DevArray<uint64_t> ck(m);
            DevArray<uint32_t> ca(m);
            DevArray<unsigned long long> n_cand(1);
            SW_HIP(hipMemsetAsync(n_cand.p, 0, 8, stream));
            DevArray<unsigned long long> ehist;
            unsigned hbits = 0, hpasses = 0;
            uint32_t iters = 1;
            if (sort_keys64_is_own(m)) {
                radix_layout(2 * nb, &hbits, &hpasses);
                ehist.alloc((size_t)hpasses << hbits);
                SW_HIP(hipMemsetAsync(ehist.p, 0, ehist.bytes(), stream));
                iters = 32;
            }
            if (unsort_hold.sorted) {
                const uint32_t n_buckets = (uint32_t)((n + UNSORT_RANGE - 1) / UNSORT_RANGE);
                const uint32_t per_wg = 4;
                DevArray<uint32_t> edge_rank(2 * (size_t)n_buckets);
                hipLaunchKernelGGL(k_unsort_adj<RecArray>, dim3((n_buckets + per_wg - 1) / per_wg), dim3(1024),
                                   ehist.p ? ((size_t)hpasses << hbits) * 4 : 0, stream, unsort_hold.sorted,
                                   n, RecArray{occ.rec.p}, d_rec_asm, 0u, nb, sentinel, k0.p, ck.p, ca.p, n_cand.p,
                                   ehist.p, hbits, hpasses, 2 * nb, edge_rank.p, per_wg);
                hipLaunchKernelGGL(k_adj_bounds<RecArray>, dim3((n_buckets + 255) / 256), dim3(256), 0, stream, edge_rank.p, n_buckets,
                                   RecArray{occ.rec.p}, d_rec_asm, 0u, nb, sentinel, k0.p, ck.p, ca.p, n_cand.p, ehist.p, hbits, hpasses,
                                   2 * nb);
                unsort_hold.a.release();
                unsort_hold.b.release();
            } else {
                hipLaunchKernelGGL(k_adj_pairs<RecArray>, dim3((adj_blocks + iters - 1) / iters), dim3(256), 0, stream, RecArray{occ.rec.p},
                                   rank.p, d_rec_asm, 0u, n, nb, sentinel, k0.p, ck.p, ca.p, n_cand.p, ehist.p, hbits, hpasses, 2 * nb, iters);
            }
            SW_HIP(hipGetLastError());
            edges_from_pairs(k0.p, k1.p, m, sentinel, nb, ab, ck.p, ca.p, n_cand.p, 0, parts.hash.p, stream, ix, (hipEvent_t) nullptr,
                             ehist.p);
        } else {
            DevArray<uint32_t> v0(m), v1(m);
            hipLaunchKernelGGL(k_adj_keys, dim3(adj_blocks), dim3(256), 0, stream, occ.rec.p, rank.p, d_rec_asm, n, nb,
                               sentinel, k0.p, v0.p);
            SW_HIP(hipGetLastError());
            edges_from_adjacency(k0.p, k1.p, v0.p, v1.p, m, sentinel, nb, parts.hash.p, stream, ix);
        }
    }
    if (ix.n_edges == 0) ix.edges.alloc(0);
    if (forked) {
        const uint64_t err = pen.active ? penalty_finish(pen) : 0;
        SW_HIP(hipStreamWaitEvent(stream, ev[5], 0));
        alloc_join(side);
        if (err) raise(SW_ERR_RUNTIME, "internal error: inconsistent occurrence order in device index (%llu)",
                       (unsigned long long)err);
    }
    SW_HIP(hipEventRecord(ev[3], stream));
    SW_HIP(hipEventSynchronize(ev[3]));
    float ms = 0.f;
    SW_HIP(hipEventElapsedTime(&ms, ev[0], ev[1]));
    ix.timings.nodes_ms = ms;
    ix.timings.counts_ms = 0;
    if (forked) {
        SW_HIP(hipEventElapsedTime(&ms, ev[4], ev[5]));
        ix.timings.counts_ms = ms;
    }
    SW_HIP(hipEventElapsedTime(&ms, ev[2], ev[3]));
    ix.timings.edges_ms = ms;
}

void index_occ_rows(const sw_index &ix, uint64_t rec_offset, uint64_t *d_rows, hipStream_t stream)
{
    if (ix.n_kmers == 0) return;
    DevArray<uint32_t> start(ix.n_nodes);
    hipLaunchKernelGGL(k_node_starts, dim3(blocks_for(ix.n_nodes)), dim3(TPB), 0, stream, ix.nodes.p, ix.n_nodes, start.p);
    hipLaunchKernelGGL(k_occ_rows, dim3(blocks_for(ix.n_kmers)), dim3(TPB), 0, stream, ix.kmers.p, ix.nodes.p, start.p,
                       ix.n_nodes, ix.n_kmers, rec_offset, d_rows);
    SW_HIP(hipGetLastError());
    SW_HIP(hipStreamSynchronize(stream));
}

void index_splits(const sw_index &ix, const uint64_t *node_bounds, const uint64_t *edge_bounds, uint32_t n_bounds,
                  uint64_t *occ_split, uint64_t *edge_split, hipStream_t stream)
{
    if (n_bounds == 0) return;
    DevArray<uint64_t> nb(n_bounds), eb(n_bounds), os(n_bounds), es(n_bounds);
    SW_HIP(hipMemcpyAsync(nb.p, node_bounds, n_bounds * 8, hipMemcpyHostToDevice, stream));
    SW_HIP(hipMemcpyAsync(eb.p, edge_bounds, n_bounds * 8, hipMemcpyHostToDevice, stream));
    hipLaunchKernelGGL(k_lower_bounds, dim3(blocks_for(n_bounds)), dim3(TPB), 0, stream, ix.nodes.p, ix.n_nodes, ix.n_kmers,
                       ix.edges.p, ix.n_edges, nb.p, eb.p, n_bounds, os.p, es.p);
    SW_HIP(hipGetLastError());
    SW_HIP(hipMemcpyAsync(occ_split, os.p, n_bounds * 8, hipMemcpyDeviceToHost, stream));
    SW_HIP(hipMemcpyAsync(edge_split, es.p, n_bounds * 8, hipMemcpyDeviceToHost, stream));
    SW_HIP(hipStreamSynchronize(stream));
}

void merge_build(const uint64_t *d_occ_rows, uint64_t n, const uint64_t *d_edge_rows, uint64_t m, uint64_t kmer_base,
                 const uint32_t *d_rec_asm, uint64_t n_records, const uint8_t *d_is_target, uint64_t n_targets,
                 uint64_t n_non_targets, hipStream_t stream, sw_index &ix, uint32_t *d_rank_out)
{
    if (n > occ_cap() || m > occ_cap()) raise_occ_cap(std::max<uint64_t>(n, m), "rows");
    ix.n_kmers = n;
    ix.kmers.alloc(n);
    ix.n_nodes = 0;
    ix.n_edges = 0;
    const bool slice = d_rank_out && m == 0 && d_rec_asm && n_records && !SW_TEST_GETENV("SEQWIN_AMD_CHECK_ORDER");
    if (n) {
        PaySort ps;
        const char *order = SW_TEST_GETENV("SEQWIN_AMD_ORDER");
        if (sort_pairs_is_own(n, 32) && !SW_TEST_GETENV("SEQWIN_AMD_SORT_KEYBITS") && !(order && !strcmp(order, "copy"))) {
            ps.rows_src = d_occ_rows;
        } else {
            ps.key_a.alloc(n);
            ps.pay_a.alloc(n);
            hipLaunchKernelGGL(k_rows_to_pay, dim3(blocks_for(n)), dim3(TPB), 0, stream, d_occ_rows, n, ps.key_a.p, ps.pay_a.p);
            SW_HIP(hipGetLastError());
        }
        DevArray<uint32_t> rec_flag;
        DevArray<unsigned long long> tbits, nbits;
        bool marked = false;
        if (d_rank_out && d_rec_asm && n_records) {
            rec_flag.alloc(n_records);
            hipLaunchKernelGGL(k_rec_flag, dim3(blocks_for(n_records)), dim3(TPB), 0, stream, d_rec_asm,
                               slice ? d_is_target : (const uint8_t *)nullptr, n_records, rec_flag.p);
            SW_HIP(hipGetLastError());
        }
        const bool bits = slice && d_is_target;
        NodeParts parts;
        const uint64_t base = slice ? kmer_base : 0;
        group_occurrences(ps, n, base, rec_flag.p, stream, ix, d_rank_out, bits ? &tbits : nullptr,
                          bits ? &nbits : nullptr, rec_flag.p ? &marked : nullptr, nullptr, &parts);
        ix.ranks_marked = marked;
        if (bits) finish_nodes(ix, parts, base, base + n, tbits.p, nbits.p, 1.0 / (double)n_targets, 1.0 / (double)n_non_targets, stream);
        else finish_nodes(ix, parts, base, base + n, nullptr, nullptr, 0.0, 0.0, stream);
        SW_HIP(hipStreamSynchronize(stream));
    } else {
        ix.nodes.alloc(0);
        ix.ranks_marked = d_rec_asm && n_records;
    }
    if (slice) {
        ix.edges.alloc(0);
        return;
    }
    PenaltyJob pen;
    Event ev_nodes(false), ev_pen(false);
    hipStream_t side = nullptr;
    if (d_is_target && ix.n_nodes) {
        side = side_stream();
        alloc_fork(side);
        SW_HIP(hipEventRecord(ev_nodes, stream));
        SW_HIP(hipStreamWaitEvent(side, ev_nodes, 0));
        penalty_launch(ix.kmers.p, n, ix.nodes.p, ix.n_nodes, d_rec_asm, n_records, d_is_target, n_targets, n_non_targets,
                       side, pen);
        SW_HIP(hipEventRecord(ev_pen, side));
    }
    ix.n_edges = 0;
    if (m) {
        DevArray<uint64_t> k0(m), k1(m), f(m), sd(m), wt(m);
        DevArray<uint32_t> v0(m), v1(m);
        hipLaunchKernelGGL(k_strided_copy, dim3(blocks_for(m)), dim3(TPB), 0, stream, d_edge_rows, 3u, 1u, m, k0.p);
        hipLaunchKernelGGL(k_iota, dim3(blocks_for(m)), dim3(TPB), 0, stream, v0.p, m);
        uint64_t *keys = k0.p, *keys_alt = k1.p;
        uint32_t *vals = v0.p, *vals_alt = v1.p;
        sort_pairs(keys, keys_alt, vals, vals_alt, m, 0, 64, stream);
        hipLaunchKernelGGL(k_gather_col, dim3(blocks_for(m)), dim3(TPB), 0, stream, d_edge_rows, 3u, 0u, vals, m, keys);
        sort_pairs(keys, keys_alt, vals, vals_alt, m, 0, 64, stream);
        hipLaunchKernelGGL(k_gather_col, dim3(blocks_for(m)), dim3(TPB), 0, stream, d_edge_rows, 3u, 0u, vals, m, f.p);
        hipLaunchKernelGGL(k_gather_col, dim3(blocks_for(m)), dim3(TPB), 0, stream, d_edge_rows, 3u, 1u, vals, m, sd.p);
        hipLaunchKernelGGL(k_gather_col, dim3(blocks_for(m)), dim3(TPB), 0, stream, d_edge_rows, 3u, 2u, vals, m, wt.p);
        SW_HIP(hipGetLastError());
        DevArray<uint32_t> ecum(m);
        inclusive_sum(rocprim::make_transform_iterator(rocprim::make_counting_iterator<uint64_t>(0), PairHeadFlag{f.p, sd.p}),
                      ecum.p, m, (uint32_t)0, stream);
        inclusive_sum(wt.p, wt.p, m, (uint64_t)0, stream);
        uint32_t n_edges = 0;
        SW_HIP(hipMemcpyAsync(&n_edges, ecum.p + (m - 1), 4, hipMemcpyDeviceToHost, stream));
        SW_HIP(hipStreamSynchronize(stream));
        ix.n_edges = n_edges;
        ix.edges.alloc(n_edges);
        DevArray<uint64_t> edge_start(n_edges);
        hipLaunchKernelGGL(k_merge_edge_heads, dim3(blocks_for(m)), dim3(TPB), 0, stream, f.p, sd.p, ecum.p, m, edge_start.p);
        hipLaunchKernelGGL(k_merge_edges, dim3(blocks_for(n_edges)), dim3(TPB), 0, stream, f.p, sd.p, wt.p, edge_start.p,
                           (uint64_t)n_edges, m, ix.edges.p);
        SW_HIP(hipGetLastError());
        SW_HIP(hipStreamSynchronize(stream));
    } else {
        ix.edges.alloc(0);
    }
    if (pen.active) {
        const uint64_t err = penalty_finish(pen);
        SW_HIP(hipStreamWaitEvent(stream, ev_pen, 0));
        alloc_join(side);
        if (err) raise(SW_ERR_RUNTIME, "internal error: inconsistent occurrence order in merged index (%llu)",
                       (unsigned long long)err);
    }
    if (kmer_base && ix.n_nodes) {
        hipLaunchKernelGGL(k_rebase_nodes, dim3(blocks_for(ix.n_nodes)), dim3(TPB), 0, stream, ix.nodes.p, ix.n_nodes,
                           kmer_base);
        SW_HIP(hipGetLastError());
        SW_HIP(hipStreamSynchronize(stream));
    }
}

namespace {
constexpr int PART_ROWS = 32;
constexpr uint32_t PART_BUCKETS = 32;

struct PartArgs;
__device__ __forceinline__ uint32_t owner_of(const PartArgs &P, uint64_t kx);
struct TupleSrc {
    const uint64_t *hash, *kmer;
    uint64_t rec_off;
    __device__ uint32_t owner(const PartArgs &P, uint64_t i) const { return owner_of(P, hash[i]); }
    __device__ void row(uint64_t i, uint64_t &r0, uint64_t &r1) const { r0 = hash[i]; r1 = kmer[i] + (rec_off << 32); }
};
struct RowSrc {
    const uint64_t *rows;
    __device__ uint32_t owner(const PartArgs &P, uint64_t i) const { return owner_of(P, rows[2 * i]); }
    __device__ void row(uint64_t i, uint64_t &r0, uint64_t &r1) const { r0 = rows[2 * i]; r1 = rows[2 * i + 1]; }
};

struct KeySrc {
    const uint64_t *rows;
    __device__ uint32_t owner(const PartArgs &P, uint64_t i) const { return owner_of(P, rows[i]); }
    __device__ void row(uint64_t i, uint64_t &r0, uint64_t &r1) const { r0 = rows[i]; r1 = 0; }
};

struct PartArgs {
    uint64_t n;
    uint64_t bounds[16];
    uint32_t n_bounds;
    uint64_t drop_key;
    uint32_t has_drop;
    uint32_t n_waves;
    uint32_t cols;
};

}
struct PartState {
    PartArgs args;
    DevArray<uint32_t> offs;
    uint64_t rec_off = 0;
    bool valid = false;
};
void part_state_delete(PartState *p) { delete p; }
uint32_t occ_partition_owners(const OrderedOcc &occ) { return occ.part && occ.part->valid ? occ.part->args.n_bounds + 1 : 0u; }
namespace {

struct OwnedKeySrc {
    const uint64_t *rows;
    const uint8_t *own;
    uint32_t n_owners;
    __device__ uint32_t owner(const PartArgs &, uint64_t i) const { const uint8_t o = own[i]; return o == OWNER_DROP ? n_owners : o; }
    __device__ void row(uint64_t i, uint64_t &r0, uint64_t &r1) const { r0 = rows[i]; r1 = 0; }
};
struct OwnedPairSrc {
    const uint64_t *key_;
    const uint32_t *asm_;
    const uint8_t *own;
    __device__ uint32_t owner(const PartArgs &, uint64_t i) const { return own[i]; }
    __device__ void row(uint64_t i, uint64_t &r0, uint64_t &r1) const { r0 = key_[i]; r1 = asm_[i]; }
};

__device__ __forceinline__ uint32_t owner_of(const PartArgs &P, uint64_t kx)
{
    uint32_t o = 0;
    for (uint32_t j = 0; j < P.n_bounds; ++j) o += (P.bounds[j] <= kx) ? 1u : 0u;
    if (P.has_drop && kx == P.drop_key) o = P.n_bounds + 1;
    return o;
}

// ... 620 lines not shown
```

Before: 496.3.

## Use per-block head counts from sort repair to replace decoupled lookback in node grouping

The sort-repair kernels now track how many run heads fall into each descent block, so each node tile's exclusive node offset can be read from a precomputed prefix of these counts. A new COUNTED variant of k_nodes takes its tile index from blockIdx, reads its base from that prefix, and skips the ticket atomic, the tile_state memset and the serial lookback chain. It is used only when the repair reports exact counts and the fused unsort route is active. The cost is extra atomics and bookkeeping in the repair kernels, more template instantiations, and a mismatch check that feeds the order-guard fallback.

```diff
diff --git a/seqwin_amd/csrc/index.hip b/seqwin_amd/csrc/index.hip
--- a/seqwin_amd/csrc/index.hip
+++ b/seqwin_amd/csrc/index.hip
@@ -106,6 +106,13 @@
     SW_HIP(rocprim::inclusive_scan(nullptr, tmp_bytes, in, out, n, rocprim::plus<T>(), stream));
     tmp.alloc(tmp_bytes);
     SW_HIP(rocprim::inclusive_scan(tmp.p, tmp_bytes, in, out, n, rocprim::plus<T>(), stream));
+}
+
+template <class F>
+void pick_bool(bool v, F f)
+{
+    if (v) f(std::true_type{});
+    else f(std::false_type{});
 }
 
 template <class InIt, class OutIt, class T>
@@ -192,9 +199,17 @@
 #endif
 constexpr int NODES_ROWS = SW_NODES_ROWS;
 constexpr int NODES_THREADS = 1024;
-constexpr int NODES_WAVES = NODES_THREADS / 64;
 constexpr uint32_t NODES_ROW = NODES_THREADS * 2;
 constexpr uint32_t NODES_TILE = NODES_ROW * NODES_ROWS;
+#ifndef SW_NODES_C_THREADS
+#define SW_NODES_C_THREADS 1024
+#endif
+#ifndef SW_NODES_C_ROWS
+#define SW_NODES_C_ROWS 4
+#endif
+constexpr int NODES_C_THREADS = SW_NODES_C_THREADS, NODES_C_ROWS = SW_NODES_C_ROWS;
+constexpr uint32_t NODES_C_TILE = NODES_C_THREADS * 2 * NODES_C_ROWS;
+constexpr uint32_t DESC_BLOCK = 1024;
 constexpr uint32_t UNSORT_BITS = 14;
 constexpr uint32_t UNSORT_RANGE = 1u << UNSORT_BITS;
 constexpr bool UNSORT_FUSED_DEFAULT = true;
@@ -216,14 +231,15 @@
 constexpr uint32_t RANK_REP = 0x80000000u;
 constexpr uint8_t OWNER_DROP = 0xFF;
 constexpr uint32_t NODES_DIGITS = 256;
+template <uint32_t TILE>
 struct NodesScat {
-    uint64_t stage[NODES_TILE];
+    uint64_t stage[TILE];
     unsigned long long goff[NODES_DIGITS];
     uint32_t cnt[NODES_DIGITS];
     uint32_t lstart[NODES_DIGITS];
 };
-template <bool BITS, bool REP, bool SCAT = false>
-__global__ __launch_bounds__(NODES_THREADS) void k_nodes(const uint32_t *__restrict__ key32, const OccPay *__restrict__ pay, uint64_t n,
+template <bool BITS, bool REP, bool SCAT = false, bool COUNTED = false, int THREADS = NODES_THREADS, int ROWS = NODES_ROWS>
+__global__ __launch_bounds__(THREADS) void k_nodes(const uint32_t *__restrict__ key32, const OccPay *__restrict__ pay, uint64_t n,
                                                uint64_t base, const uint32_t *__restrict__ rec_flag, sw_kmer *__restrict__ kmers,
                                                uint64_t *__restrict__ node_hash, uint32_t *__restrict__ node_start,
                                                uint32_t *__restrict__ rank_direct,
@@ -231,28 +247,34 @@
                                                unsigned long long *__restrict__ tbits, unsigned long long *__restrict__ nbits,
                                                unsigned long long *__restrict__ tile_state, uint32_t *__restrict__ ticket,
                                                uint32_t *__restrict__ n_nodes_out, uint32_t *__restrict__ order_bad,
-                                               unsigned long long *__restrict__ cursor, uint32_t dig_shift, uint32_t dig_mask)
-{
+                                               unsigned long long *__restrict__ cursor, uint32_t dig_shift, uint32_t dig_mask,
+                                               const unsigned long long *__restrict__ block_base = nullptr)
+{
+    constexpr int WAVES = THREADS / 64;
+    constexpr uint32_t ROW = THREADS * 2, TILE = ROW * ROWS;
+    static_assert(TILE % DESC_BLOCK == 0, "a counted tile starts at a block of the descent sweep");
     __shared__ uint32_t s_tile, s_excl;
-    __shared__ uint32_t s_row[NODES_ROWS * NODES_WAVES];
-    static_assert(NODES_ROWS * NODES_WAVES <= 128, "the (row, wave) group counts are scanned by one wave, two per lane");
+    __shared__ uint32_t s_row[ROWS * WAVES];
+    static_assert(ROWS * WAVES <= 128, "the (row, wave) group counts are scanned by one wave, two per lane");
     const uint32_t lane = threadIdx.x & 63u, wave = threadIdx.x >> 6;
-    NodesScat *sc = nullptr;
+    NodesScat<TILE> *sc = nullptr;
     if constexpr (SCAT) {
-        __shared__ NodesScat s_scat;
+        __shared__ NodesScat<TILE> s_scat;
         sc = &s_scat;
         if (threadIdx.x < NODES_DIGITS) sc->cnt[threadIdx.x] = 0;
     }
-    if (threadIdx.x == 0) s_tile = atomicAdd(ticket, 1u);
-    __syncthreads();
-    const uint32_t tile = s_tile;
-    const uint64_t s0 = (uint64_t)tile * NODES_TILE;
-    uint32_t k[NODES_ROWS][2], within[NODES_ROWS], headm = 0, prec[NODES_ROWS];
-    OccPay p[NODES_ROWS][2];
+    if constexpr (!COUNTED) {
+        if (threadIdx.x == 0) s_tile = atomicAdd(ticket, 1u);
+    }
+    if constexpr (!COUNTED || SCAT) __syncthreads();
+    const uint32_t tile = COUNTED ? blockIdx.x : s_tile;
+    const uint64_t s0 = (uint64_t)tile * TILE;
+    uint32_t k[ROWS][2], within[ROWS], headm = 0, prec[ROWS];
+    OccPay p[ROWS][2];
     unsigned long long misorder = 0;
 #pragma unroll
-    for (int r = 0; r < NODES_ROWS; ++r) {
-        const uint64_t s = s0 + (uint64_t)r * NODES_ROW + 2 * threadIdx.x;
+    for (int r = 0; r < ROWS; ++r) {
+        const uint64_t s = s0 + (uint64_t)r * ROW + 2 * threadIdx.x;
         k[r][0] = k[r][1] = 0;
         p[r][0] = p[r][1] = OccPay{0, 0, 0, 0};
         if (s + 1 < n) {
@@ -291,17 +313,17 @@
         within[r] = (uint32_t)__popcll(b0 & lt) + (uint32_t)__popcll(b1 & lt);
         if (h0) headm |= 1u << (2 * r);
         if (h1) headm |= 2u << (2 * r);
-        if (lane == 0) s_row[r * NODES_WAVES + wave] = (uint32_t)__popcll(b0) + (uint32_t)__popcll(b1);
+        if (lane == 0) s_row[r * WAVES + wave] = (uint32_t)__popcll(b0) + (uint32_t)__popcll(b1);
     }
     if (misorder && lane == 0) atomicAdd(order_bad, (uint32_t)__popcll(misorder));
-    uint32_t drank[NODES_ROWS][2];
+    uint32_t drank[ROWS][2];
     if constexpr (SCAT) {
 #pragma unroll
-        for (int r = 0; r < NODES_ROWS; ++r)
+        for (int r = 0; r < ROWS; ++r)
 #pragma unroll
             for (int e = 0; e < 2; ++e) {
                 drank[r][e] = 0;
-                if (s0 + (uint64_t)r * NODES_ROW + 2 * threadIdx.x + e < n)
+                if (s0 + (uint64_t)r * ROW + 2 * threadIdx.x + e < n)
                     drank[r][e] = atomicAdd(&sc->cnt[(p[r][e].idx >> dig_shift) & dig_mask], 1u);
             }
     }
@@ -327,7 +349,7 @@
         }
     }
     if (wave == 0) {
-        constexpr uint32_t GROUPS = NODES_ROWS * NODES_WAVES;
+        constexpr uint32_t GROUPS = ROWS * WAVES;
         const uint32_t c0 = (2 * lane < GROUPS) ? s_row[2 * lane] : 0u, c1 = (2 * lane + 1 < GROUPS) ? s_row[2 * lane + 1] : 0u;
         uint32_t incl = c0 + c1;
         for (uint32_t d = 1; d < 64; d <<= 1) {
@@ -337,10 +359,16 @@
         const uint32_t total = __shfl(incl, 63, 64);
         if (2 * lane < GROUPS) s_row[2 * lane] = incl - c0 - c1;
         if (2 * lane + 1 < GROUPS) s_row[2 * lane + 1] = incl - c1;
-        if (lane == 0)
+        if (!COUNTED && lane == 0)
             __hip_atomic_store(&tile_state[tile], (tile == 0 ? TS_INC : TS_AGG) | total, __ATOMIC_RELAXED, __HIP_MEMORY_SCOPE_AGENT);
         uint32_t excl = 0;
-        if (tile) {
+        if constexpr (COUNTED) {
+            constexpr uint64_t PER = TILE / DESC_BLOCK;
+            const uint64_t n_blocks = (n + DESC_BLOCK - 1) / DESC_BLOCK, b0 = (uint64_t)tile * PER;
+            excl = (uint32_t)(block_base[b0] >> 32);
+            const uint32_t next = (uint32_t)(block_base[min(b0 + PER, n_blocks)] >> 32);
+            if (lane == 0 && next - excl != total) atomicAdd(order_bad, 1u);
+        } else if (tile) {
             int64_t look = (int64_t)tile - 1;
             for (;;) {
                 const int64_t idx = look - lane;
@@ -365,23 +393,23 @@
         }
         if (lane == 0) {
             s_excl = excl;
-            if (s0 + NODES_TILE >= n) *n_nodes_out = excl + total;
+            if (s0 + TILE >= n) *n_nodes_out = excl + total;
         }
     }
     __syncthreads();
     const uint32_t excl = s_excl;
     if constexpr (SCAT) {
 #pragma unroll
-        for (int r = 0; r < NODES_ROWS; ++r)
+        for (int r = 0; r < ROWS; ++r)
 #pragma unroll
             for (int e = 0; e < 2; ++e) drank[r][e] += sc->lstart[(p[r][e].idx >> dig_shift) & dig_mask];
     }
 #pragma unroll
-    for (int r = 0; r < NODES_ROWS; ++r) {
-        const uint64_t s = s0 + (uint64_t)r * NODES_ROW + 2 * threadIdx.x;
+    for (int r = 0; r < ROWS; ++r) {
+        const uint64_t s = s0 + (uint64_t)r * ROW + 2 * threadIdx.x;
         const bool live0 = s < n, live1 = s + 1 < n;
         const bool h0 = (headm >> (2 * r)) & 1u, h1 = (headm >> (2 * r + 1)) & 1u;
-        const uint32_t nid0 = excl + s_row[r * NODES_WAVES + wave] + within[r] + (h0 ? 1u : 0u) - 1u;
+        const uint32_t nid0 = excl + s_row[r * WAVES + wave] + within[r] + (h0 ? 1u : 0u) - 1u;
         const uint32_t nid1 = nid0 + (h1 ? 1u : 0u);
         uint32_t w0 = nid0, w1 = nid1;
         uint32_t f0 = 0, f1 = 0, pf = 0;
@@ -457,16 +485,16 @@
         asm volatile("s_waitcnt lgkmcnt(0)" ::: "memory");
         __builtin_amdgcn_s_barrier();
         asm volatile("" ::: "memory");
-        const uint32_t cnt_tile = (uint32_t)min((uint64_t)NODES_TILE, n - s0);
-        constexpr int OUT = NODES_TILE / NODES_THREADS;
+        const uint32_t cnt_tile = (uint32_t)min((uint64_t)TILE, n - s0);
+        constexpr int OUT = TILE / THREADS;
         uint64_t word[OUT], at[OUT];
 #pragma unroll
-        for (int j = 0; j < OUT; ++j) word[j] = sc->stage[j * NODES_THREADS + threadIdx.x];
-#pragma unroll
-        for (int j = 0; j < OUT; ++j) at[j] = sc->goff[(uint32_t)(word[j] >> (32 + dig_shift)) & dig_mask] + (j * NODES_THREADS + threadIdx.x);
+        for (int j = 0; j < OUT; ++j) word[j] = sc->stage[j * THREADS + threadIdx.x];
+#pragma unroll
+        for (int j = 0; j < OUT; ++j) at[j] = sc->goff[(uint32_t)(word[j] >> (32 + dig_shift)) & dig_mask] + (j * THREADS + threadIdx.x);
 #pragma unroll
         for (int j = 0; j < OUT; ++j)
-            if (j * NODES_THREADS + threadIdx.x < cnt_tile && at[j] < n) uval[at[j]] = word[j];
+            if (j * THREADS + threadIdx.x < cnt_tile && at[j] < n) uval[at[j]] = word[j];
     }
 }
 
@@ -1617,7 +1645,6 @@
     }
 }
 
-constexpr uint32_t DESC_BLOCK = 1024;
 
 struct PayView {
     using Key = uint32_t;
@@ -1849,10 +1876,25 @@
 __device__ __forceinline__ uint32_t readlane_key(uint32_t v, uint32_t lane) { return (uint32_t)__builtin_amdgcn_readlane((int)v, (int)lane); }
 __device__ __forceinline__ uint64_t readlane_key(uint64_t v, uint32_t lane) { return readlane64(v, lane); }
 
+__device__ __forceinline__ void book_heads(unsigned long long *__restrict__ heads, uint64_t block, int d)
+{
+    if (d) atomicAdd(&heads[block], (unsigned long long)(long long)d << 32);
+}
+enum { RD_THREAD = 0, RD_WAVE, RD_GROUP, RD_CHANGED, RD_BLOCK_EDGE, RD_TILE_EDGE, RD_WORDS };
+__device__ __forceinline__ void repair_debug(unsigned long long *__restrict__ dbg, int form, uint64_t a, uint32_t len, bool changed)
+{
+    if (!dbg) return;
+    atomicAdd(&dbg[form], 1ull);
+    if (changed) atomicAdd(&dbg[RD_CHANGED], 1ull);
+    if (a / DESC_BLOCK != (a + len - 1) / DESC_BLOCK) atomicAdd(&dbg[RD_BLOCK_EDGE], 1ull);
+    if (a / NODES_TILE != (a + len - 1) / NODES_TILE) atomicAdd(&dbg[RD_TILE_EDGE], 1ull);
+}
+
 template <class View>
 __global__ __launch_bounds__(256) void k_repair_thread(const View V, typename View::Key kmask, uint64_t n, const uint32_t *__restrict__ bad_q,
                                                        const unsigned long long *__restrict__ n_desc, uint32_t *__restrict__ mid,
-                                                       uint32_t *__restrict__ n_mid, uint32_t *__restrict__ status)
+                                                       uint32_t *__restrict__ n_mid, uint32_t *__restrict__ status,
+                                                       unsigned long long *__restrict__ heads, unsigned long long *__restrict__ dbg)
 {
     constexpr uint32_t RT = REPAIR_THREAD_RUN;
     const unsigned long long D = *n_desc;
@@ -1891,6 +1933,24 @@
                     rank[i] += (ki[j] < ki[i] || (ki[j] == ki[i] && (lj < li || (lj == li && j < i)))) ? 1u : 0u;
                 }
         }
+        if (heads) {
+            const uint64_t b0 = a / DESC_BLOCK;
+            int d0 = 0, d1 = 0;
+#pragma unroll
+            for (uint32_t i = 0; i < RT; ++i)
+                if (i < len) {
+                    bool was = true, first = true;
+                    if (i) was = ki[i] != ki[i - 1] || View::low_of(vi[i]) != View::low_of(vi[i - 1]);
+#pragma unroll
+                    for (uint32_t j = 0; j < i; ++j)
+                        if (ki[j] == ki[i] && View::low_of(vi[j]) == View::low_of(vi[i])) first = false;
+                    if (was) ((a + i) / DESC_BLOCK == b0 ? d0 : d1) -= 1;
+                    if (first) ((a + rank[i]) / DESC_BLOCK == b0 ? d0 : d1) += 1;
+                }
+            book_heads(heads, b0, d0);
+            book_heads(heads, b0 + 1, d1);
+            repair_debug(dbg, RD_THREAD, a, len, d0 || d1);
+        }
 #pragma unroll
         for (uint32_t i = 0; i < RT; ++i)
             if (i < len && rank[i] != i) V.store(a + rank[i], ki[i], vi[i]);
@@ -1901,7 +1961,8 @@
 __global__ __launch_bounds__(256) void k_repair_wave(const View V, typename View::Key kmask, uint64_t n, const uint32_t *__restrict__ bad_q,
                                                      const unsigned long long *__restrict__ n_desc, const uint32_t *__restrict__ mid,
                                                      const uint32_t *__restrict__ n_mid, uint32_t *__restrict__ big,
-                                                     uint32_t *__restrict__ n_big, uint32_t *__restrict__ status)
+                                                     uint32_t *__restrict__ n_big, uint32_t *__restrict__ status,
+                                                     unsigned long long *__restrict__ heads, unsigned long long *__restrict__ dbg)
 {
     if (*n_desc > REPAIR_MAX_DESC) return;
     const uint32_t M = min(*n_mid, REPAIR_MAX_MID);
@@ -1954,10 +2015,26 @@
             li = View::low_of(vi);
         }
         uint32_t rank = 0;
+        bool first = have;
         for (uint32_t j = 0; j < len; ++j) {
             const typename View::Key kj = readlane_key(ki, j);
             const uint64_t lj = readlane64(li, j);
             rank += (kj < ki || (kj == ki && (lj < li || (lj == li && j < lane)))) ? 1u : 0u;
+            if (kj == ki && lj == li && j < lane) first = false;
+        }
+        if (heads) {
+            const typename View::Key kp = __shfl_up(ki, 1, 64);
+            const uint64_t lp = __shfl_up(li, 1, 64);
+            const bool was = have && (lane == 0 || ki != kp || li != lp);
+            const uint64_t b0 = a / DESC_BLOCK;
+            const bool was0 = (a + lane) / DESC_BLOCK == b0, now0 = (a + rank) / DESC_BLOCK == b0;
+            const int d0 = __popcll(__ballot(first && now0)) - __popcll(__ballot(was && was0));
+            const int d1 = __popcll(__ballot(first && !now0)) - __popcll(__ballot(was && !was0));
+            if (lane == 0) {
+                book_heads(heads, b0, d0);
+                book_heads(heads, b0 + 1, d1);
+                repair_debug(dbg, RD_WAVE, a, len, d0 || d1);
+            }
         }
         if (have) V.store(a + rank, ki, vi);
     }
@@ -1965,8 +2042,10 @@
 
 constexpr uint32_t REPAIR_MAX_VALUES = 12;
 template <class View>
-__global__ __launch_bounds__(256) void k_repair_sort(const View V, const uint32_t *__restrict__ n_big, const uint32_t *__restrict__ big)
-{
+__global__ __launch_bounds__(256) void k_repair_sort(const View V, const uint32_t *__restrict__ n_big, const uint32_t *__restrict__ big,
+                                                     unsigned long long *__restrict__ heads, unsigned long long *__restrict__ dbg)
+{
+    __shared__ int s_d[3];
     __shared__ typename View::Elem sv[REPAIR_MAX_RUN];
     __shared__ typename View::Key sk[REPAIR_MAX_RUN];
     __shared__ uint16_t srank[REPAIR_MAX_RUN];
@@ -1978,9 +2057,15 @@
     for (uint32_t b = blockIdx.x; b < B; b += gridDim.x) {
         const uint32_t a = big[2 * b], len = big[2 * b + 1];
         __syncthreads();
+        if (tid < 3) s_d[tid] = 0;
         for (uint32_t i = tid; i < len; i += blockDim.x) V.load(a + i, sk[i], sv[i]);
         __syncthreads();
         const uint32_t per = (len + 255u) / 256u, i0 = min(len, tid * per), i1 = min(len, i0 + per);
+        const uint32_t b0 = a / DESC_BLOCK;
+        if (heads)
+            for (uint32_t i = i0; i < i1; ++i)
+                if (i == 0 || sk[i] != sk[i - 1] || View::low_of(sv[i]) != View::low_of(sv[i - 1])) atomicSub(&s_d[(a + i) / DESC_BLOCK - b0], 1);
+        int now[3] = {0, 0, 0};
         uint32_t placed = 0;
         typename View::Key last_k = 0;
         uint64_t last_l = 0;
@@ -2040,6 +2125,12 @@
             }
             for (uint32_t i = i0; i < i1; ++i)
                 if (sk[i] == mk && View::low_of(sv[i]) == ml) srank[i] = (uint16_t)before++;
+            {
+                const uint32_t at = (a + placed) / DESC_BLOCK - b0;
+                now[0] += at == 0;
+                now[1] += at == 1;
+                now[2] += at == 2;
+            }
             placed += total;
             last_k = mk;
             last_l = ml;
@@ -2047,6 +2138,8 @@
         }
         __syncthreads();
         if (placed == len) {
+            if (heads && tid == 0)
+                for (int j = 0; j < 3; ++j) atomicAdd(&s_d[j], now[j]);
             for (uint32_t i = tid; i < len; i += blockDim.x) V.store(a + srank[i], sk[i], sv[i]);
         } else {
             for (uint32_t i = tid; i < len; i += blockDim.x) {
@@ -2054,13 +2147,21 @@
                 const typename View::Elem vi = sv[i];
                 const uint64_t li = View::low_of(vi);
                 uint32_t rank = 0;
+                bool first = true;
                 for (uint32_t j = 0; j < len; ++j) {
                     const typename View::Key kj = sk[j];
                     const uint64_t lj = View::low_of(sv[j]);
                     rank += (kj < ki || (kj == ki && (lj < li || (lj == li && j < i)))) ? 1u : 0u;
+                    if (kj == ki && lj == li && j < i) first = false;
                 }
+                if (heads && first) atomicAdd(&s_d[(a + rank) / DESC_BLOCK - b0], 1);
                 V.store(a + rank, ki, vi);
             }
+        }
+        if (heads) {
+            __syncthreads();
+            if (tid < 3) book_heads(heads, (uint64_t)b0 + tid, s_d[tid]);
+            if (tid == 0) repair_debug(dbg, RD_GROUP, a, len, s_d[0] || s_d[1] || s_d[2]);
         }
     }
 }
@@ -2068,13 +2169,15 @@
 struct RepairState {
     DevArray<unsigned long long> n_desc;
     DevArray<unsigned long long> blk_cnt, blk_off;
+    bool counted = false;
+    DevArray<unsigned long long> dbg;
     DevArray<uint32_t> slot_q, slot_k;
     DevArray<uint32_t> bad_q, mid, big, status;
 };
 
 template <class View, class Sweep>
 void enqueue_repair(const View &V, const Sweep &W, typename View::Key kmask, uint64_t n, uint32_t *bad, uint32_t cap, RepairState &r,
-                    hipStream_t stream)
+                    hipStream_t stream, bool count_heads = false)
 {
     const uint32_t n_blocks = (uint32_t)((n + DESC_BLOCK - 1) / DESC_BLOCK);
     const uint32_t max_desc = (uint32_t)std::min<uint64_t>(REPAIR_MAX_DESC, std::max<uint64_t>(n, 1));
@@ -2084,8 +2187,18 @@
     r.big.alloc(2 * (size_t)max_mid);
     r.n_desc.alloc(2);
     r.status.alloc(3);
-    r.blk_cnt.alloc(n_blocks);
-    r.blk_off.alloc(n_blocks);
+    r.blk_cnt.alloc((size_t)n_blocks + 1);
+    r.blk_off.alloc((size_t)n_blocks + 1);
+    r.counted = count_heads;
+    unsigned long long *heads = count_heads ? r.blk_cnt.p : nullptr, *dbg = nullptr;
+    if (count_heads) {
+        SW_HIP(hipMemsetAsync(r.blk_cnt.p + n_blocks, 0, 8, stream));
+        if (getenv("SEQWIN_AMD_DEBUG_NODES")) {
+            r.dbg.alloc(RD_WORDS);
+            SW_HIP(hipMemsetAsync(r.dbg.p, 0, RD_WORDS * 8, stream));
+            dbg = r.dbg.p;
+        }
+    }
     r.slot_q.alloc((size_t)n_blocks * DESC_SLOT);
     r.slot_k.alloc((size_t)n_blocks * DESC_SLOT);
     SW_HIP(hipMemsetAsync(r.status.p, 0, 12, stream));
@@ -2095,11 +2208,12 @@
     hipLaunchKernelGGL(k_list_descents<Sweep>, dim3(n_blocks), dim3(256), 0, stream, W, kmask, n, r.blk_cnt.p, r.blk_off.p,
                        n_blocks, bad, cap, r.bad_q.p, max_desc, r.n_desc.p, r.slot_q.p, r.slot_k.p);
     hipLaunchKernelGGL(k_repair_thread<View>, dim3(REPAIR_GRID), dim3(256), 0, stream, V, kmask, n, r.bad_q.p, r.n_desc.p, r.mid.p,
-                       r.status.p + 2, r.status.p);
+                       r.status.p + 2, r.status.p, heads, dbg);
     hipLaunchKernelGGL(k_repair_wave<View>, dim3(REPAIR_GRID), dim3(256), 0, stream, V, kmask, n, r.bad_q.p, r.n_desc.p,
-                       (const uint32_t *)r.mid.p, (const uint32_t *)(r.status.p + 2), r.big.p, r.status.p + 1, r.status.p);
-    hipLaunchKernelGGL(k_repair_sort<View>, dim3(REPAIR_GRID), dim3(256), 0, stream, V, r.status.p + 1, r.big.p);
+                       (const uint32_t *)r.mid.p, (const uint32_t *)(r.status.p + 2), r.big.p, r.status.p + 1, r.status.p, heads, dbg);
+    hipLaunchKernelGGL(k_repair_sort<View>, dim3(REPAIR_GRID), dim3(256), 0, stream, V, r.status.p + 1, r.big.p, heads, dbg);
     SW_HIP(hipGetLastError());
+    if (count_heads) exclusive_sum(r.blk_cnt.p, r.blk_off.p, (size_t)n_blocks + 1, 0ull, stream);
 }
 
 __global__ void k_bad_runs(const uint32_t *__restrict__ bad, uint32_t n_bad, const uint32_t *__restrict__ key32,
@@ -2171,6 +2285,7 @@
     RepairState rep;
     uint32_t cap = 0, kmask = ~0u;
     uint64_t n = 0;
+    bool heads_exact = false;
     DevArray<uint32_t> fail;
     DevArray<uint32_t> low;
     const uint64_t *rows_src = nullptr;
@@ -2192,6 +2307,7 @@
     OccPay *vals = o.pay_a.p, *vals_alt = o.pay_b.p;
     bool have_low = false;
     const bool want_low = bits == 32;
+    bool own = true;
     if (o.staged) {
         OrderedOcc &occ = *o.staged;
         StageSource S{};
@@ -2237,7 +2353,8 @@
         }
         o.fail.alloc(1);
         SW_HIP(hipMemsetAsync(o.fail.p, 0, 4, stream));
-        if (want_low && sort_pairs_is_own(n, bits)) o.low.alloc(n);
+        own = sort_pairs_is_own(n, bits);
+        if (want_low && own) o.low.alloc(n);
         have_low = sort_pairs32(keys, keys_alt, vals, vals_alt, n, bits, stream, o.fail.p, o.low.p);
         if (bits < 32) {
             hipLaunchKernelGGL(k_rot_keys, dim3(blocks_for(n)), dim3(TPB), 0, stream, keys, n, 32 - bits);
@@ -2248,8 +2365,8 @@
     o.pay = vals;
     o.cap = (uint32_t)std::min<uint64_t>(n, std::max<uint64_t>(1u << 16, n / 16));
     o.bad.alloc(o.cap);
-    if (have_low) enqueue_repair(PayView{keys, vals}, LowView{keys, o.low.p}, o.kmask, n, o.bad.p, o.cap, o.rep, stream);
-    else enqueue_repair(PayView{keys, vals}, PayView{keys, vals}, o.kmask, n, o.bad.p, o.cap, o.rep, stream);
+    if (have_low) enqueue_repair(PayView{keys, vals}, LowView{keys, o.low.p}, o.kmask, n, o.bad.p, o.cap, o.rep, stream, own);
+    else enqueue_repair(PayView{keys, vals}, PayView{keys, vals}, o.kmask, n, o.bad.p, o.cap, o.rep, stream, own);
 }
 
 bool sort_pay_settle(PaySort &o, unsigned long long D, uint32_t status, hipStream_t stream)
@@ -2303,14 +2420,23 @@
 uint64_t settle_sort(PaySort &ps, hipStream_t stream)
 {
     uint32_t status = 0, failed = 0;
-    unsigned long long dh[2] = {0, 0};
+    unsigned long long dh[2] = {0, 0}, total = 0, dbg[RD_WORDS] = {};
+    const uint64_t n_blocks = (ps.n + DESC_BLOCK - 1) / DESC_BLOCK;
     SW_HIP(hipMemcpyAsync(&status, ps.rep.status.p, 4, hipMemcpyDeviceToHost, stream));
     SW_HIP(hipMemcpyAsync(dh, ps.rep.n_desc.p, 16, hipMemcpyDeviceToHost, stream));
+    if (ps.rep.counted) SW_HIP(hipMemcpyAsync(&total, ps.rep.blk_off.p + n_blocks, 8, hipMemcpyDeviceToHost, stream));
+    if (ps.rep.dbg.p) SW_HIP(hipMemcpyAsync(dbg, ps.rep.dbg.p, sizeof dbg, hipMemcpyDeviceToHost, stream));
     if (ps.fail.p) SW_HIP(hipMemcpyAsync(&failed, ps.fail.p, 4, hipMemcpyDeviceToHost, stream));
     SW_HIP(hipStreamSynchronize(stream));
     check_sort_failed(failed);
     sort_pay_settle(ps, dh[0], status, stream);
-    return dh[1];
+    ps.heads_exact = ps.rep.counted && (dh[0] == 0 || status == 0);
+    if (ps.rep.dbg.p)
+        fprintf(stderr, "[repair] %llu descents, runs: thread %llu, wave %llu, workgroup %llu; head count changed in %llu, across a block edge %llu, "
+                        "across a tile edge %llu; run heads %llu -> %llu (%s)\n",
+                dh[0], dbg[RD_THREAD], dbg[RD_WAVE], dbg[RD_GROUP], dbg[RD_CHANGED], dbg[RD_BLOCK_EDGE], dbg[RD_TILE_EDGE], dh[1], total >> 32,
+                ps.heads_exact ? "exact" : "left to the general repair");
+    return ps.heads_exact ? total >> 32 : dh[1];
 }
 
 struct UnsortHold {
@@ -2380,7 +2506,7 @@
 }
 uint32_t group_occurrences(PaySort &ps, uint64_t n, uint64_t base, const uint32_t *rec_flag, hipStream_t stream, sw_index &ix,
                            uint32_t *rank_out, DevArray<unsigned long long> *tbits, DevArray<unsigned long long> *nbits,
-                           bool *rep_marked = nullptr, UnsortHold *hold = nullptr, NodeParts *parts = nullptr)
+                           bool *rep_marked = nullptr, UnsortHold *hold = nullptr, NodeParts *parts = nullptr, bool allow_counted = false)
 {
     sort_pay(n, stream, ps);
     const uint64_t node_cap = settle_sort(ps, stream);
@@ -2401,8 +2527,11 @@
         tbits->alloc((n + 63) / 64);
         nbits->alloc((n + 63) / 64);
     }
-    const unsigned blocks = (unsigned)((n + NODES_TILE - 1) / NODES_TILE);
-    DevArray<unsigned long long> tile_state(blocks);
+    const unsigned blocks = (unsigned)((n + NODES_TILE - 1) / NODES_TILE), cblocks = (unsigned)((n + NODES_C_TILE - 1) / NODES_C_TILE);
+    DevArray<unsigned long long> tile_state;
+    const char *base_env = SW_TEST_GETENV("SEQWIN_AMD_NODES_BASE");
+    const bool never_counted = base_env && !strcmp(base_env, "lookback"), always_counted = base_env && !strcmp(base_env, "counted");
+    const bool can_count = allow_counted && ps.heads_exact && !never_counted;
     DevArray<uint32_t> words(4);
     uint32_t back[3] = {0, 0, 0};
     if (rank_out && !direct) uv1.alloc(n);
@@ -2412,29 +2541,33 @@
     if (const char *e = SW_TEST_GETENV("SEQWIN_AMD_UNSORT_FUSED")) want_fused = atoi(e) != 0;
     UnsortPerm perm;
     const char *route = !rank_out ? "none" : direct ? "direct" : nbit <= UNSORT_BITS ? "one bucket" : "sort";
+    bool counted = false;
     for (int attempt = 0;; ++attempt) {
-        SW_HIP(hipMemsetAsync(tile_state.p, 0, (size_t)blocks * 8, stream));
         SW_HIP(hipMemsetAsync(words.p, 0, 16, stream));
         const bool fused = want_fused && rank_out && !direct && nbit > UNSORT_BITS && sort_keys64_is_own(n) &&
                            radix_unsort_perm_begin(perm, n, UNSORT_BITS, nbit, stream);
-        {
-            auto launch = [&](auto kern) {
-                hipLaunchKernelGGL(kern, dim3(blocks), dim3(NODES_THREADS), 0, stream, ps.key32, ps.pay, n, base, rec_flag, ix.kmers.p,
-                                   np.hash.p, np.start.p, direct ? rank_out : (uint32_t *)nullptr, fused ? uv1.p : uv0.p,
-                                   bits ? tbits->p : (unsigned long long *)nullptr, bits ? nbits->p : (unsigned long long *)nullptr,
-                                   tile_state.p, words.p, words.p + 1, words.p + 3, fused ? perm.cur_a.p : (unsigned long long *)nullptr,
-                                   fused ? perm.low_bits + 8 : 0u, fused ? (1u << perm.hi_bits) - 1u : 0u);
-            };
-            if (fused) {
-                if (bits && rep) launch(k_nodes<true, true, true>);
-                else if (bits) launch(k_nodes<true, false, true>);
-                else if (rep) launch(k_nodes<false, true, true>);
-                else launch(k_nodes<false, false, true>);
-            } else if (bits && rep) launch(k_nodes<true, true>);
-            else if (bits) launch(k_nodes<true, false>);
-            else if (rep) launch(k_nodes<false, true>);
-            else launch(k_nodes<false, false>);
-        }
+        counted = can_count && attempt == 0 && (fused || always_counted);
+        if (!counted) {
+            if (!tile_state.p) tile_state.alloc(blocks);
+            SW_HIP(hipMemsetAsync(tile_state.p, 0, (size_t)blocks * 8, stream));
+        }
+        pick_bool(bits, [&](auto B) {
+            pick_bool(rep, [&](auto R) {
+                pick_bool(fused, [&](auto S) {
+                    pick_bool(counted, [&](auto C) {
+                        constexpr bool c = decltype(C)::value;
+                        hipLaunchKernelGGL((k_nodes<decltype(B)::value, decltype(R)::value, decltype(S)::value, c, c ? NODES_C_THREADS : NODES_THREADS,
+                                                    c ? NODES_C_ROWS : NODES_ROWS>),
+                                           dim3(c ? cblocks : blocks), dim3(c ? NODES_C_THREADS : NODES_THREADS), 0, stream, ps.key32, ps.pay, n, base,
+                                           rec_flag, ix.kmers.p, np.hash.p, np.start.p, direct ? rank_out : (uint32_t *)nullptr,
+                                           fused ? uv1.p : uv0.p, bits ? tbits->p : (unsigned long long *)nullptr,
+                                           bits ? nbits->p : (unsigned long long *)nullptr, tile_state.p, words.p, words.p + 1, words.p + 3,
+                                           fused ? perm.cur_a.p : (unsigned long long *)nullptr, fused ? perm.low_bits + 8 : 0u,
+                                           fused ? (1u << perm.hi_bits) - 1u : 0u, (const unsigned long long *)ps.rep.blk_off.p);
+                    });
+                });
+            });
+        });
         SW_HIP(hipGetLastError());
         if (rank_out && !direct) {
             uint64_t *v = uv0.p;
@@ -2457,8 +2590,8 @@
         SW_HIP(hipMemcpyAsync(back, words.p + 1, 12, hipMemcpyDeviceToHost, stream));
         SW_HIP(hipStreamSynchronize(stream));
         if (getenv("SEQWIN_AMD_DEBUG_NODES"))
-            fprintf(stderr, "[nodes] %llu occurrences (indices of %u bits), attempt %d: unsort route %s, %u nodes, order guard %u\n",
-                    (unsigned long long)n, nbit, attempt, route, back[0], back[2]);
+            fprintf(stderr, "[nodes] %llu occurrences (indices of %u bits), attempt %d: unsort route %s, nodes base %s, %u nodes, order guard %u\n",
+                    (unsigned long long)n, nbit, attempt, route, counted ? "counted" : "lookback", back[0], back[2]);
         if (back[2] == 0) break;
         if (attempt)
             raise(SW_ERR_RUNTIME, "internal error: the node sort is still out of order after the rocPRIM re-sort (%u places)", back[2]);
@@ -3237,7 +3370,7 @@
         ps.pay_a = std::move(occ.pay);
         if (occ.staged) ps.staged = &occ;
         group_occurrences(ps, n, 0, rec_flag.p, stream, ix, by_table ? nullptr : rank.p, bits ? &tbits : nullptr,
-                          bits ? &nbits : nullptr, pair_edges ? &rep_marked : nullptr, pair_edges ? &unsort_hold : nullptr, &parts);
+                          bits ? &nbits : nullptr, pair_edges ? &rep_marked : nullptr, pair_edges ? &unsort_hold : nullptr, &parts, true);
         if (!bits || by_table) {
             finish_nodes(ix, parts, 0, n, nullptr, nullptr, 0.0, 0.0, stream);
             if (by_table) ranks_from_table(ix, occ.hash.p, n, stream, rank.p);
```

Result: no change. 498.8 (median of 6 runs) (+0.5%).
